# hzxie/Stereo-3D-Reconstruction

Hardware: NVIDIA B200
Metric: stereo pairs/sec Stereo2Voxel fwd (higher is better)
Workload: dtype bf16

## Files before the change

### include/s3d.h

```cpp
#ifndef S3D_H_
#define S3D_H_

#include <stdint.h>

#ifdef __cplusplus
extern "C" {
#endif

#define S3D_OK                0
#define S3D_ERR_INVALID      -1
#define S3D_ERR_CUDA         -2
#define S3D_ERR_UNSUPPORTED  -3

#define S3D_DTYPE_F32   0
#define S3D_DTYPE_BF16  1
#define S3D_DTYPE_BF16X2 2

#define S3D_ACT_NONE     0
#define S3D_ACT_RELU     1
#define S3D_ACT_LEAKY    2
#define S3D_ACT_SIGMOID  3
#define S3D_ACT_TANH     4

#define S3D_MAX_TAPS 64

typedef struct S3dConvParams {
  int32_t N, iD, iH, iW, Cin;
  int32_t oD, oH, oW, Cout;
  int32_t sz, sy, sx;
  int32_t ntaps, n_classes;
  int8_t  dz[S3D_MAX_TAPS], dy[S3D_MAX_TAPS], dx[S3D_MAX_TAPS];
  int64_t osN, osD, osH, osW;
  int64_t osC;
  int64_t os_lo;
  int32_t omz, omy, omx;
  int32_t cout_store;
  int32_t in_dtype, out_dtype;
  int32_t act;  float act_param;
  int32_t tw, th, td, tn;
  int32_t bn;
  const float* proj_w;
  int32_t proj_channel, proj_act;
  const void* w_nstack;
} S3dConvParams;

const char* s3d_version(void);
const char* s3d_last_error(void);
int s3d_device_check(int dev);
int s3d_set_knob(const char* name, int value);
int s3d_get_knob(const char* name);

int s3d_conv_igemm(const S3dConvParams* p, const void* in, const void* w, const float* bias,
                   const void* residual, void* out, void* stream);
int s3d_conv_direct(const S3dConvParams* p, const void* in, const void* w, const float* bias,
                    const void* residual, void* out, void* stream);

int s3d_conv2d_halo(const void* in, const void* w, const float* bias, const void* residual, void* out, int nimg, int h, int wd,
                    int cin, int cout, int64_t osN, int64_t osH, int64_t osW, int relu, void* stream);

int s3d_pack_image(const float* img, const float* disp, float disp_scale, void* out,
                   int B, int H, int W, int Cpad, int out_dtype, void* stream);

int s3d_pack_image_u8(const uint8_t* img, const float* disp, float disp_scale, float img_scale, void* out,
                      int B, int H, int W, int Cpad, int out_dtype, void* stream);

int s3d_conv_first(const void* img, int img_u8, const float* disp, float disp_scale, const void* w, const float* bias,
                   void* out, int B, int H, int W, int cin, int cin_pad, int cout_pad, int dtype, int act,
                   float act_param, void* stream);

int s3d_conv_concat_volume(const S3dConvParams* p, const void* feat, int feat_pitch, int feat_pad, const float* bias,
                           void* out, void* stream);
int s3d_conv_concat_volume_ro(const S3dConvParams* p, const void* feat, int feat_pitch, int feat_pad, const void* w_refonce,
                              const float* bias, void* out, void* stream);
int s3d_concat_gonce_assemble(const float* maps_l, const float* maps_r, const float* edge_l, const float* edge_r,
                              const float* bias, void* out, int B, int D, int h, int w, int map_w, int out_dtype, void* stream);
int s3d_map_conv(const void* in, const void* w, float* out, int nimg, int h, int in_w, int ow, int off, int ntx, int cout,
                 int dtype, void* stream);
int s3d_cost_volume_concat(const void* feat, void* vol, int B, int h, int w, int C, int D,
                           int dtype, void* stream);
int s3d_soft_argmin(const float* cost, float* disp, int N, int D, int h, int w, float sign,
                    void* stream);
int s3d_tap_gather_soft_argmin(const float* taps, float* disp, float* cost_out, int N, int D, int h, int w,
                               int tap_stride, float sign, void* stream);
int s3d_cls_soft_argmin(const void* x, const void* w_taps, float* disp, int N, int D, int h, int w, int C,
                        float sign, void* stream);
int64_t s3d_conv_cls_workspace_bytes(int N, int D, int h, int w);
int s3d_conv_cls_soft_argmin(const S3dConvParams* p, const void* in, const float* bias, const void* w_taps, void* workspace,
                             float* disp, float sign, void* stream);
int s3d_corr_soft_argmin(const void* feat, float* disp, float* cost_out, int B, int h, int w,
                         int C, int c_real, int D, int dtype, void* stream);
int s3d_upsample_disp(const float* disp_q, float* disp, int N, int h, int w, int H, int W,
                      float scale, void* stream);
int s3d_upsample_disp_eval(const float* disp_q, float* disp, const float* gt, const float* thresholds, int T,
                           float max_gt, long long* stats, int B, int h, int w, int H, int W, float scale, void* stream);
int s3d_upsample_disp_lr(const float* disp_q, float* disp, uint8_t* lr_mask, float lr_thresh, const float* gt,
                         const float* thresholds, int T, float max_gt, long long* disp_stats, long long* lr_stats,
                         int B, int h, int w, int H, int W, float scale, void* stream);

int s3d_latent_to_vox(const void* x, void* out, int N, int H, int W, int C, int L, int dtype,
                      void* stream);
int s3d_avg_pool(const void* x, void* out, int N, int H, int W, int C, int L, int dtype,
                 void* stream);
int s3d_depth_to_space(const void* in, void* out, const float* proj_w, int proj_act, int N, int d, int h, int w,
                       int Cpad, int dtype, void* stream);
int s3d_split_tf32(const float* x, float* hi, float* lo, int64_t n, void* stream);
int s3d_split_bf16(const float* x, void* out, int64_t npix, int C, void* stream);
int s3d_unsplit_bf16(const void* x, float* out, int64_t npix, int C, void* stream);
int s3d_fuse_views(const void* score, int64_t score_stride, const void* vol, int64_t vol_stride,
                   int dtype, float* fused, int B, int V, int nvox, const uint8_t* gt,
                   const float* thresholds, int T, long long* iou, int64_t score_lo, int64_t vol_lo, void* stream);

int s3d_chamfer_forward(const float* xyz1, const float* xyz2, float* dist1, int32_t* idx1,
                        float* dist2, int32_t* idx2, int B, int N, int M, void* stream);
int64_t s3d_chamfer_workspace_bytes(int B, int N, int M);
int s3d_chamfer_forward_ws(const float* xyz1, const float* xyz2, float* dist1, int32_t* idx1,
                           float* dist2, int32_t* idx2, int B, int N, int M, void* workspace,
                           int64_t workspace_bytes, void* stream);
int s3d_chamfer_eval(const float* xyz1, const float* xyz2, float* dist1, int32_t* idx1, float* dist2, int32_t* idx2,
                     int B, int N, int M, const float* tau, int T, long long* stats,
                     void* workspace, int64_t workspace_bytes, void* stream);

int s3d_fma_probe(float* sink, int iters, int64_t* fma_count, void* stream);

#ifdef __cplusplus
}
#endif
#endif
```

### stereo_3d_reconstruction_b200/csrc/common.cuh

```cuda
#pragma once
#include <cuda_runtime.h>
#include <cuda_bf16.h>
#include <stdint.h>
#include <stdio.h>
#include "../../include/s3d.h"

namespace s3d {

void set_error(const char* fmt, ...);

#define S3D_CHECK_ARG(cond, ...)                         \
  do {                                                   \
    if (!(cond)) {                                       \
      s3d::set_error(__VA_ARGS__);                       \
      return S3D_ERR_INVALID;                            \
    }                                                    \
  } while (0)

#define S3D_CUDA(expr)                                                              \
  do {                                                                              \
    cudaError_t _e = (expr);                                                        \
    if (_e != cudaSuccess) {                                                        \
      s3d::set_error("%s:%d %s -> %s", __FILE__, __LINE__, #expr, cudaGetErrorString(_e)); \
      return S3D_ERR_CUDA;                                                          \
    }                                                                               \
  } while (0)

#define S3D_LAUNCH_CHECK() S3D_CUDA(cudaGetLastError())

int num_sms();

struct Knobs {
  int no_scatter;
  int scatter_tps3;
  int scatter_no_pair;
  int scatter_ring;
  int scatter_res_transpose;
  int scatter_no_transpose;
  int scatter_generic;
  int no_corr_tc;
  int scatter_zsplit;
  int igemm_ts1;
  int igemm_one_cta;
  int scatter_one_cta;
  int no_conv_first_tc;
  int chamfer_sym;
  int chamfer_sym_r;
  int scatter_no_rm;
};
Knobs& knobs();

static inline int ceil_div(int a, int b) { return (a + b - 1) / b; }
static inline int64_t ceil_div64(int64_t a, int64_t b) { return (a + b - 1) / b; }

namespace {
constexpr int kMaxThresh = 8;
struct Thresh { float t[kMaxThresh]; };
}

template <typename T> __device__ __forceinline__ float to_f32(T v);
template <> __device__ __forceinline__ float to_f32<float>(float v) { return v; }
template <> __device__ __forceinline__ float to_f32<__nv_bfloat16>(__nv_bfloat16 v) { return __bfloat162float(v); }

template <typename T> __device__ __forceinline__ T from_f32(float v);
template <> __device__ __forceinline__ float from_f32<float>(float v) { return v; }
template <> __device__ __forceinline__ __nv_bfloat16 from_f32<__nv_bfloat16>(float v) { return __float2bfloat16_rn(v); }

__device__ __forceinline__ float fmax_nan(float a, float b) { float d; asm("max.NaN.f32 %0, %1, %2;" : "=f"(d) : "f"(a), "f"(b)); return d; }
__device__ __forceinline__ float fmin_nan(float a, float b) { float d; asm("min.NaN.f32 %0, %1, %2;" : "=f"(d) : "f"(a), "f"(b)); return d; }

__device__ __forceinline__ float apply_act(float v, int act, float a) {
  switch (act) {
    case S3D_ACT_RELU:    return fmax_nan(v, 0.f);
    case S3D_ACT_LEAKY:   return v > 0.f ? v : v * a;
    case S3D_ACT_SIGMOID: return 1.f / (1.f + expf(-v));
    case S3D_ACT_TANH:    return a * tanhf(v);
    default:              return v;
  }
}

static __device__ __noinline__ float apply_act_slow(float v, int act, float a) { return apply_act(v, act, a); }

}
```

### stereo_3d_reconstruction_b200/csrc/conv_scatter.cu

```cuda
#include "conv_scatter.cuh"

namespace s3d {
using namespace scatter;

bool conv_scatter_eligible(const S3dConvParams* p) {
  const int esz = p->in_dtype == S3D_DTYPE_F32 ? 4 : 2;
  const bool split = p->in_dtype == S3D_DTYPE_BF16X2;
  if (!p->w_nstack || knobs().no_scatter) return false;
  if (split && (p->out_dtype != S3D_DTYPE_BF16X2 || p->Cin > 64 || (p->Cout != 16 && p->Cout != 32 && p->Cout != 64) ||
                p->cout_store != p->Cout)) return false;
  if (!split && p->out_dtype == S3D_DTYPE_BF16X2) return false;
  if (p->n_classes != 1 || p->sx != 1 || p->sy != 1 || p->sz != 1 || p->ntaps != 27) return false;
  if (p->omx != 1 || p->omy != 1 || p->omz != 1 || p->osC != 1 || p->proj_w) return false;
  if (p->oD != p->iD || p->oH != p->iH || p->oW != p->iW) return false;
  for (int t = 0; t < 27; ++t)
    if (p->dz[t] != t / 9 - 1 || p->dy[t] != (t % 9) / 3 - 1 || p->dx[t] != t % 3 - 1) return false;
  const int cin_bytes = (split ? 2 : 1) * p->Cin * esz;
  if (split && cin_bytes == 32) return false;
  if (cin_bytes != 32 && cin_bytes != 64 && cin_bytes != 128 && cin_bytes != 256) return false;
  if (p->Cout > 64 || p->Cout % 16 != 0) return false;
  return true;
}

int conv_scatter_launch(const S3dConvParams* p_in, const void* in, const float* bias, const void* residual, void* out,
                        cudaStream_t stream) {
  const S3dConvParams& p = *p_in;
  const bool tf32 = p.in_dtype == S3D_DTYPE_F32;
  const bool split = p.in_dtype == S3D_DTYPE_BF16X2;
  const int esz = tf32 ? 4 : 2;
  const int cin_phys = split ? 2 * p.Cin : p.Cin;
  S3D_CHECK_ARG(p.cout_store >= 1 && p.cout_store <= p.Cout, "scatter: cout_store");
  ScArgs a;
  memset(&a, 0, sizeof(a));
  a.p = p;  a.bias = bias;  a.residual = residual;  a.out = out;
  a.split = split ? 1 : 0;
  a.os_lo = p.os_lo ? p.os_lo : (int64_t)p.Cout;
  a.nchunks = cin_phys * esz == 256 ? 2 : 1;
  a.row_bytes = cin_phys * esz / a.nchunks;
  a.kc = cin_phys / a.nchunks;
  a.chunk_stride = (kPlaneRows * a.row_bytes + 1023) / 1024 * 1024;
  a.slot_bytes = a.nchunks * a.chunk_stride;
  a.cp = p.Cout;
  a.tps = spec_tps(a.row_bytes, a.cp);
  if (knobs().scatter_tps3 && a.tps == 9) a.tps = 3;
  a.cols_x = ceil_div(p.oW, kTX);  a.cols_y = ceil_div(p.oH, kTY);
  int64_t total = (int64_t)p.N * a.cols_x * a.cols_y;
  S3D_CHECK_ARG(total > 0 && total < (1ll << 31), "scatter: column count out of range");
  a.nz = 1;  a.zc = p.oD;  a.dl = p.oD;
  {
    const int sms = num_sms();
    int nz = knobs().scatter_zsplit > 0 ? knobs().scatter_zsplit : (knobs().scatter_zsplit < 0 ? 1 : (int)(sms / total));
    if (nz > p.oD / 4) nz = p.oD / 4;
    if (nz > 1) {
      a.zc = ceil_div(p.oD, nz);
      a.nz = ceil_div(p.oD, a.zc);
      a.dl = a.zc + 2;
      if (a.nz > 1) total *= a.nz; else { a.nz = 1; a.zc = p.oD; a.dl = p.oD; }
    }
  }
  a.total_cols = (int)total;
  int grid = num_sms();
  a.pair = ((3 * a.cp / 2) % 8 == 0 && total >= 2 && grid >= 2 && !knobs().scatter_no_pair) ? 1 : 0;
  bool fast_ok;
  {
    const int oesz = p.out_dtype == S3D_DTYPE_F32 ? 4 : 2;
    const bool simple_act = p.act == S3D_ACT_NONE || p.act == S3D_ACT_RELU || p.act == S3D_ACT_LEAKY;
    auto aligned = [&](const void* q) { return (reinterpret_cast<uintptr_t>(q) & 15) == 0; };
    auto dense16 = [&](int64_t st) { return (st * oesz) % 16 == 0; };
    fast_ok = simple_act && bias != nullptr && p.cout_store == p.Cout && aligned(out) && aligned(residual) &&
              dense16(p.osW) && dense16(p.osH) && dense16(p.osD) && dense16(p.osN) && p.osW < (1ll << 24) &&
              (split || !knobs().scatter_no_transpose);
  }
  const bool two = fast_ok && a.pair && !tf32 && !split && a.nchunks == 1 && p.out_dtype == S3D_DTYPE_BF16 && residual == nullptr &&
                   spec_kernel(a.row_bytes, a.cp, false, p.act == S3D_ACT_RELU, true) != nullptr && total > grid &&
                   !knobs().scatter_generic && !knobs().scatter_one_cta && !knobs().scatter_tps3 && !knobs().scatter_ring;
  if (two) grid *= 2;
  if (a.pair) {
    if ((int64_t)grid > total) grid = (int)((total + 1) / 2 * 2);
    grid -= grid % 2;
    a.ncols_max = (int)((total + grid - 1) / grid);
  } else if ((int64_t)grid > total) grid = (int)total;
  const int w_rows = a.pair ? 3 * a.cp / 2 : 3 * a.cp;
  a.w_tx = a.tps * w_rows * a.row_bytes;
  a.w_bytes = (a.w_tx + 1023) / 1024 * 1024;
  const int budget = two ? 110 * 1024 : 227 * 1024 - 1024 - 512;
  int ring = (budget - 4 * a.w_bytes) / a.slot_bytes;
  if (ring > kMaxRing) ring = kMaxRing;
  if (ring < 2) ring = 2;
  if (a.row_bytes == 128 && ring > (a.pair && a.nchunks == 1 ? 3 : 2)) ring = a.pair && a.nchunks == 1 ? 3 : 2;
  if (const int r = knobs().scatter_ring) { if (r >= 2 && r <= kMaxRing) ring = r; }
  a.ring = ring;
  a.w_stages = (budget - a.ring * a.slot_bytes) / a.w_bytes;
  if (a.w_stages > kMaxW) a.w_stages = kMaxW;
  S3D_CHECK_ARG(a.w_stages >= 2, "scatter: not enough shared memory for the weight ring");
  a.idesc = ptx::make_instr_desc(tf32 ? 2 : 1, a.pair ? 256 : 128, 3 * a.cp);
  a.res_direct = !knobs().scatter_res_transpose;
  {
    auto dense16 = [&](int64_t st) { return (st * 2) % 16 == 0; };
    a.fast_store = fast_ok;
    if (split) {
      S3D_CHECK_ARG(a.fast_store && dense16(a.os_lo) && a.os_lo >= p.Cout,
                    "scatter (split operands): needs a bias, a none / ReLU / LeakyReLU activation and 16-byte aligned out / residual / strides");
      a.res_direct = 1;
    }
  }

  const CUtensorMapSwizzle sw = a.row_bytes == 128 ? CU_TENSOR_MAP_SWIZZLE_128B
                              : a.row_bytes == 64 ? CU_TENSOR_MAP_SWIZZLE_64B : CU_TENSOR_MAP_SWIZZLE_32B;
  CUtensorMap map_x, map_w;
  cuuint32_t box[5] = {(cuuint32_t)a.kc, kHX, kHY, 1, 1};
  cuuint32_t estr[5] = {1, 1, 1, 1, 1};
  int rc = encode_act_map(&map_x, in, esz, tf32, cin_phys, p.iW, p.iH, p.iD, p.N, box, estr, sw);
  if (rc != S3D_OK) return rc;
  rc = encode_weight_map(&map_w, p.w_nstack, esz, tf32, cin_phys, 3 * a.cp, 36, a.kc, w_rows, sw, a.tps);
  if (rc != S3D_OK) return rc;

  const bool rm = residual != nullptr && a.pair && !tf32 && !split && a.nchunks == 1 && a.row_bytes == 128 && a.cp == 64 &&
                  p.out_dtype == S3D_DTYPE_BF16 && a.fast_store && a.tps == 1 && (p.act == S3D_ACT_RELU || p.act == S3D_ACT_NONE) &&
                  p.osW == 64 && p.osH == (int64_t)p.oW * 64 && p.osD == (int64_t)p.oH * p.osH && p.osN == (int64_t)p.oD * p.osD &&
                  !knobs().scatter_no_rm && !knobs().scatter_generic;
  if (rm) {
    const int extra = kResBytes + 32 * 128;
    a.w_stages = (budget - a.ring * a.slot_bytes - extra) / a.w_bytes;
    if (a.w_stages > kMaxW) a.w_stages = kMaxW;
    S3D_CHECK_ARG(a.w_stages >= 3, "scatter: not enough shared memory for the residual stage");
    CUtensorMap map_r;
    cuuint32_t rbox[5] = {64, kTX, kTY, 1, 1};
    rc = encode_act_map(&map_r, residual, 2, false, 64, p.oW, p.oH, p.oD, p.N, rbox, estr, CU_TENSOR_MAP_SWIZZLE_128B);
    if (rc != S3D_OK) return rc;
    a.residual = nullptr;
    const int smem_rm = a.ring * a.slot_bytes + a.w_stages * a.w_bytes + extra + 1024;
    KernFnR kr = rm_kernel(p.act == S3D_ACT_RELU);
    S3D_CUDA(cudaFuncSetAttribute(kr, cudaFuncAttributeMaxDynamicSharedMemorySize, smem_rm));
    cudaLaunchConfig_t cfg;
    memset(&cfg, 0, sizeof(cfg));
    cfg.gridDim = dim3(grid);  cfg.blockDim = dim3(kThreads);  cfg.dynamicSmemBytes = smem_rm;  cfg.stream = stream;
    cudaLaunchAttribute attr;
    attr.id = cudaLaunchAttributeClusterDimension;
    attr.val.clusterDim.x = 2;  attr.val.clusterDim.y = 1;  attr.val.clusterDim.z = 1;
    cfg.attrs = &attr;  cfg.numAttrs = 1;
    S3D_CUDA(cudaLaunchKernelEx(&cfg, kr, map_x, map_w, map_r, a));
    S3D_LAUNCH_CHECK();
    return S3D_OK;
  }

  const int smem_bytes = a.ring * a.slot_bytes + a.w_stages * a.w_bytes + 1024;
  KernFn kern = a.pair ? (tf32 ? conv_scatter_kernel<true, true> : conv_scatter_kernel<false, true>)
                       : (tf32 ? conv_scatter_kernel<true, false> : conv_scatter_kernel<false, false>);
  if (split) {
    const bool lean = a.pair && a.tps == spec_tps(a.row_bytes, a.cp) && !knobs().scatter_generic;
    kern = split_kernel(lean, a.pair != 0, cin_phys * esz, a.cp, residual != nullptr, p.act == S3D_ACT_RELU);
  }
  else if (a.pair && !tf32 && a.nchunks == 1 && p.out_dtype == S3D_DTYPE_BF16 && a.fast_store && a.tps == spec_tps(a.row_bytes, a.cp) &&
      !knobs().scatter_generic) {
    const bool relu = p.act == S3D_ACT_RELU;
    if (KernFn k = spec_kernel(a.row_bytes, a.cp, residual != nullptr, relu, two && a.fast_store)) kern = k;
    else if (two) { set_error("scatter: the two-CTA kernel needs the coalesced store path"); return S3D_ERR_INVALID; }
  }
  S3D_CUDA(cudaFuncSetAttribute(kern, cudaFuncAttributeMaxDynamicSharedMemorySize, smem_bytes));
  if (a.pair) {
    cudaLaunchConfig_t cfg;
    memset(&cfg, 0, sizeof(cfg));
    cfg.gridDim = dim3(grid);  cfg.blockDim = dim3(kThreads);  cfg.dynamicSmemBytes = smem_bytes;  cfg.stream = stream;
    cudaLaunchAttribute attr;
    attr.id = cudaLaunchAttributeClusterDimension;
    attr.val.clusterDim.x = 2;  attr.val.clusterDim.y = 1;  attr.val.clusterDim.z = 1;
    cfg.attrs = &attr;  cfg.numAttrs = 1;
    S3D_CUDA(cudaLaunchKernelEx(&cfg, kern, map_x, map_w, a));
  } else {
    kern<<<grid, kThreads, smem_bytes, stream>>>(map_x, map_w, a);
  }
  S3D_LAUNCH_CHECK();
  return S3D_OK;
}

}
```

### stereo_3d_reconstruction_b200/csrc/conv_scatter.cuh

```cuda
#pragma once
#include <cuda.h>
#include <stdlib.h>
#include <string.h>
#include "common.cuh"
#include "ptx.cuh"
#include "epilogue.cuh"

namespace s3d {
namespace scatter {

constexpr int kThreads = 384;
constexpr int kTX = 8, kHX = kTX + 2;
constexpr int kTY = 32, kHY = kTY + 2;
constexpr int kTileY = 16;
constexpr int kPlaneRows = kHX * kHY;
constexpr int kMaxRing = 6;
constexpr int kMaxW = 12;
constexpr int kTmemCols = 512;
constexpr int kTileCols = 256;

struct ScArgs {
  S3dConvParams p;
  const float* bias;
  const void* residual;
  void* out;
  int row_bytes;
  int kc;
  int nchunks;
  int chunk_stride;
  int slot_bytes;
  int ring;
  int cp;
  int tps;
  int w_stages, w_bytes, w_tx;
  int cols_x, cols_y, total_cols;
  int pair;
  int ncols_max;
  uint32_t idesc;
  int fast_store;
  int res_direct;
  int split;
  int64_t os_lo;
  int nz, zc, dl;
};

struct ScCtrl {
  uint64_t plane_full[kMaxRing], plane_empty[kMaxRing];
  uint64_t w_full[kMaxW], w_empty[kMaxW];
  uint64_t acc_full[2], acc_empty[2];
  uint64_t res_full, res_empty;
  uint32_t tmem_base;
};

struct ScRes {
  const CUtensorMap* map_r;
  uint32_t res_u32;
  uint32_t ident_u32;
  uint32_t bar_rf, bar_re;
  uint32_t idesc_r;
  int cp;
};
constexpr int kResBytes = 256 * 128;

struct Col { int n, y0, x0, zb; };

__device__ __forceinline__ Col decode_col(const ScArgs& a, int c) {
  Col r;
  r.zb = 0;
  if (a.nz > 1) { r.zb = (c % a.nz) * a.zc - 1;  c /= a.nz; }
  r.x0 = (c % a.cols_x) * kTX;  c /= a.cols_x;
  r.y0 = (c % a.cols_y) * kTY;  c /= a.cols_y;
  r.n = c;
  return r;
}

__device__ __forceinline__ int cta_cols(const ScArgs& a) {
  return a.pair ? a.ncols_max : (a.total_cols - (int)blockIdx.x + (int)gridDim.x - 1) / (int)gridDim.x;
}

__device__ __forceinline__ uint64_t desc_hi(uint32_t sbo, int row_bytes) {
  const uint64_t layout = row_bytes == 128 ? 2ull : (row_bytes == 64 ? 4ull : 6ull);
  return (static_cast<uint64_t>(sbo >> 4) << 32) | (1ull << 46) | (layout << 61);
}
__device__ __forceinline__ uint32_t desc_lo(uint32_t addr) { return ((addr & 0x3FFFF) >> 4) | (1u << 16); }

template <int TPS, bool kPair, int NK = 1, bool kRM = false>
__device__ __forceinline__ void sc_produce(const ScArgs& a, ScCtrl& ctrl, uint32_t planes_u32, uint32_t w_u32,
                                           const CUtensorMap* map_x, const CUtensorMap* map_w, const ScRes* rs = nullptr) {
  constexpr int G = 9 * NK / TPS;
  const uint32_t bar_pf = ptx::smem_u32(&ctrl.plane_full[0]), bar_pe = ptx::smem_u32(&ctrl.plane_empty[0]);
  const uint32_t bar_wf = ptx::smem_u32(&ctrl.w_full[0]), bar_we = ptx::smem_u32(&ctrl.w_empty[0]);
  const int D = a.dl, ring = a.ring, w_stages = a.w_stages, ncols = cta_cols(a);
  const int slot_bytes = a.slot_bytes, w_bytes = a.w_bytes, w_tx = a.w_tx;
  const int crank = kPair ? (int)ptx::cluster_ctarank() : 0;
  const bool leader = crank == 0;
  const int w_row0 = kPair ? crank * (3 * a.cp / 2) : 0;
  const int plane_tx = NK * kPlaneRows * a.row_bytes;
  const int kc = a.kc, chunk_stride = a.chunk_stride;
  int ws = 0;  uint32_t wphase = 0;
  int pslot = 0;  uint32_t pphase = 0;
  int pci = 0, pj = 0, issued = 0;
  Col pc = decode_col(a, blockIdx.x);
  auto issue_plane = [&](bool blocking) -> bool {
    if (pci >= ncols) return false;
    const uint32_t be = bar_pe + 8 * pslot, bf = bar_pf + 8 * pslot;
    if (blocking) ptx::mbar_wait_u32(be, pphase ^ 1);
    else if (!ptx::mbar_test_wait_u32(be, pphase ^ 1)) return false;
    if (ptx::elect_one()) {
      if (kPair) {
        if (leader) ptx::mbar_arrive_expect_tx_u32(bf, 2 * plane_tx);
#pragma unroll
        for (int ch = 0; ch < NK; ++ch)
          ptx::tma_load_5d_2sm_u32(planes_u32 + pslot * slot_bytes + ch * chunk_stride, map_x, bf, ch * kc, pc.x0 - 1, pc.y0 - 1, pc.zb + pj, pc.n);
      } else {
        ptx::mbar_arrive_expect_tx_u32(bf, plane_tx);
#pragma unroll
        for (int ch = 0; ch < NK; ++ch)
          ptx::tma_load_5d_u32(planes_u32 + pslot * slot_bytes + ch * chunk_stride, map_x, bf, ch * kc, pc.x0 - 1, pc.y0 - 1, pc.zb + pj, pc.n);
      }
    }
    __syncwarp();
    ++issued;
    if (++pslot == ring) { pslot = 0; pphase ^= 1; }
    if (++pj == D) {
      pj = 0;  ++pci;
      if (pci < ncols) pc = decode_col(a, blockIdx.x + pci * gridDim.x);
    }
    return true;
  };
  int gp = 0;
  [[maybe_unused]] uint32_t rphase = 0;
  [[maybe_unused]] auto load_res = [&](const Col& rc, int p) {
    ptx::mbar_wait_u32(rs->bar_re, rphase ^ 1);
    if (ptx::elect_one()) {
      if (kPair) {
        if (leader) ptx::mbar_arrive_expect_tx_u32(rs->bar_rf, 2 * kResBytes);
        ptx::tma_load_5d_2sm_u32(rs->res_u32, rs->map_r, rs->bar_rf, 0, rc.x0, rc.y0, rc.zb + p, rc.n);
      } else {
        ptx::mbar_arrive_expect_tx_u32(rs->bar_rf, kResBytes);
        ptx::tma_load_5d_u32(rs->res_u32, rs->map_r, rs->bar_rf, 0, rc.x0, rc.y0, rc.zb + p, rc.n);
      }
    }
    __syncwarp();
    rphase ^= 1;
  };
  for (int ci = 0; ci < ncols; ++ci) {
    int rot = 3;
    [[maybe_unused]] const Col rc = decode_col(a, blockIdx.x + ci * gridDim.x);
    if constexpr (kRM) load_res(rc, 0);
    for (int p = 0; p < D; ++p, ++gp) {
      while (issued <= gp) issue_plane(true);
      const int ahead = gp + ring;
#pragma unroll
      for (int g = 0; g < G; ++g) {
        if (issued < ahead) issue_plane(false);
        const uint32_t be = bar_we + 8 * ws, bf = bar_wf + 8 * ws;
        ptx::mbar_wait_u32(be, wphase ^ 1);
        if (ptx::elect_one()) {
          const int tap = rot * 9 + (NK == 2 ? g / 2 : g * TPS), c0 = NK == 2 ? (g & 1) * kc : 0;
          if (kPair) {
            if (leader) ptx::mbar_arrive_expect_tx_u32(bf, 2 * w_tx);
            ptx::tma_load_3d_2sm_u32(w_u32 + ws * w_bytes, map_w, bf, c0, w_row0, tap);
          } else {
            ptx::mbar_arrive_expect_tx_u32(bf, w_tx);
            ptx::tma_load_3d_u32(w_u32 + ws * w_bytes, map_w, bf, c0, 0, tap);
          }
        }
        __syncwarp();
        if (++ws == w_stages) { ws = 0; wphase ^= 1; }
      }
      if constexpr (kRM) { if (p + 1 < D) load_res(rc, p + 1); }
      rot = (p == 0) ? 1 : (rot == 2 ? 0 : rot + 1);
    }
  }
}

struct ScIssue {
  uint32_t tmem_base, planes_u32, w_u32;
  uint32_t bar_pf, bar_pe, bar_wf, bar_we, bar_af, bar_ae;
  uint64_t x_hi, w_hi;
  int slot_bytes, w_bytes, w_stages, ring;
  uint32_t rb16, tap_step, tile_off, chunk_step;
  uint32_t idesc;
  int D, ncols;
};

template <bool kPair>
__device__ __forceinline__ void sc_commit(uint32_t bar) {
  if (kPair) ptx::tc_commit_2sm_u32(bar, 3);
  else       ptx::tc_commit_u32(bar);
}

template <bool kTF32, bool kPair>
__device__ __forceinline__ void sc_mma(uint32_t d_tmem, uint64_t ad, uint64_t bd, uint32_t idesc, uint32_t acc) {
  if (kPair) { if (kTF32) ptx::mma_tf32_2sm(d_tmem, ad, bd, idesc, acc); else ptx::mma_bf16_2sm(d_tmem, ad, bd, idesc, acc); }
  else       { if (kTF32) ptx::mma_tf32(d_tmem, ad, bd, idesc, acc);     else ptx::mma_bf16(d_tmem, ad, bd, idesc, acc); }
}

template <bool kTF32, int TPS, int kPer, bool kPair, int NK, bool kSplit>
__device__ __forceinline__ void sc_issue_group(const ScIssue& z, uint32_t d_tmem, uint64_t xdesc, uint64_t wdesc, int g,
                                               uint32_t first) {
#pragma unroll
  for (int tt = 0; tt < TPS; ++tt) {
    const int kyx = NK == 2 ? g / 2 : g * TPS + tt;
    const uint32_t xrow = ((kyx / 3) * kHX + (kyx % 3)) * z.rb16;
    if constexpr (!kSplit) {
      const uint32_t xoff = xrow + (NK == 2 ? (g & 1) * z.chunk_step : 0u);
#pragma unroll
      for (int k = 0; k < kPer; ++k) {
        const uint32_t acc = (g == 0 && tt == 0 && k == 0) ? first : 1u;
        sc_mma<kTF32, kPair>(d_tmem, xdesc + xoff + 2 * k, wdesc + tt * z.tap_step + 2 * k, z.idesc, acc);
      }
    } else if constexpr (NK == 2) {
      if ((g & 1) == 0) {
#pragma unroll
        for (int k = 0; k < kPer; ++k)
          sc_mma<kTF32, kPair>(d_tmem, xdesc + xrow + 2 * k, wdesc + 2 * k, z.idesc, (g == 0 && k == 0) ? first : 1u);
#pragma unroll
        for (int k = 0; k < kPer; ++k)
          sc_mma<kTF32, kPair>(d_tmem, xdesc + xrow + z.chunk_step + 2 * k, wdesc + 2 * k, z.idesc, 1u);
      } else {
#pragma unroll
        for (int k = 0; k < kPer; ++k)
          sc_mma<kTF32, kPair>(d_tmem, xdesc + xrow + 2 * k, wdesc + 2 * k, z.idesc, 1u);
      }
    } else {
      const uint64_t wd = wdesc + tt * z.tap_step;
#pragma unroll
      for (int k = 0; k < kPer; ++k)
        sc_mma<kTF32, kPair>(d_tmem, xdesc + xrow + 2 * k, wd + 2 * k, z.idesc, (g == 0 && tt == 0 && k == 0) ? first : 1u);
#pragma unroll
      for (int k = 0; k < kPer; ++k)
        sc_mma<kTF32, kPair>(d_tmem, xdesc + xrow + 2 * (kPer + k), wd + 2 * k, z.idesc, 1u);
#pragma unroll
      for (int k = 0; k < kPer; ++k)
        sc_mma<kTF32, kPair>(d_tmem, xdesc + xrow + 2 * k, wd + 2 * (kPer + k), z.idesc, 1u);
    }
  }
}

template <bool kPair, int CP>
__device__ __forceinline__ void sc_res_mma(const ScRes& rs, uint32_t d_tmem, uint64_t adesc, uint64_t idd) {
#pragma unroll
  for (int k = 0; k < CP / 16; ++k) sc_mma<false, kPair>(d_tmem, adesc + 2 * k, idd + 2 * k, rs.idesc_r, 1u);
}

template <bool kTF32, int TPS, int kPer, bool kPair, int NK = 1, bool kSplit = false, bool kRM = false, int kTP = kTileCols>
__device__ __forceinline__ void sc_issue(const ScIssue& z, const ScRes* rs = nullptr) {
  constexpr int G = 9 * NK / TPS;
  int ws = 0;  uint32_t wphase = 0;
  int pw = 0;  uint32_t pwphase = 0;
  uint32_t aphase = 0;
  [[maybe_unused]] uint32_t rphase = 0;
  [[maybe_unused]] uint64_t rdesc = 0, idd = 0;
  if constexpr (kRM) {
    const uint64_t hi = desc_hi(8 * 128, 128);
    rdesc = hi | desc_lo(rs->res_u32);
    idd = hi | desc_lo(rs->ident_u32);
  }
  const uint32_t w_lo0 = desc_lo(z.w_u32), w_lo_step = z.w_bytes >> 4;
  const uint32_t x_lo0 = desc_lo(z.planes_u32), x_lo_step = z.slot_bytes >> 4;
  const uint32_t d0 = z.tmem_base, d1 = z.tmem_base + kTP;
  for (int ci = 0; ci < z.ncols; ++ci) {
    for (int p = 0; p < z.D; ++p) {
      ptx::mbar_wait_u32(z.bar_pf + 8 * pw, pwphase);
      const uint64_t xd0 = z.x_hi | (x_lo0 + pw * x_lo_step);
      const uint64_t xd1 = xd0 + z.tile_off;
      const uint32_t first = p == 0 ? 0u : 1u;
      int ws_prev = 0;
#pragma unroll
      for (int g = 0; g <= G; ++g) {
        if (g < G) {
          ptx::mbar_wait_u32(z.bar_wf + 8 * ws, wphase);
          if (g == 0) ptx::mbar_wait_u32(z.bar_ae, aphase ^ 1);
          ptx::tc_fence_after();
          const uint64_t wd = z.w_hi | (w_lo0 + ws * w_lo_step);
          if constexpr (kRM) { if (g == G / 2) { ptx::mbar_wait_u32(rs->bar_rf, rphase); ptx::tc_fence_after(); } }
          if (ptx::elect_one()) {
            sc_issue_group<kTF32, TPS, kPer, kPair, NK, kSplit>(z, d0, xd0, wd, g, first);
            if constexpr (kRM) { if (g == G / 2) sc_res_mma<kPair, 64>(*rs, d0 + (uint32_t)(p % 3) * rs->cp, rdesc, idd); }
            if (g == G - 1) sc_commit<kPair>(z.bar_af);
          }
          __syncwarp();
        }
        if (g >= 1) {
          if (g == 1) { ptx::mbar_wait_u32(z.bar_ae + 8, aphase ^ 1); ptx::tc_fence_after(); }
          const uint64_t wd = z.w_hi | (w_lo0 + ws_prev * w_lo_step);
          if (ptx::elect_one()) {
            sc_issue_group<kTF32, TPS, kPer, kPair, NK, kSplit>(z, d1, xd1, wd, g - 1, first);
            sc_commit<kPair>(z.bar_we + 8 * ws_prev);
            if constexpr (kRM) {
              if (g == G / 2 + 1) {
                sc_res_mma<kPair, 64>(*rs, d1 + (uint32_t)(p % 3) * rs->cp, rdesc + (128 * 128 >> 4), idd);
                sc_commit<kPair>(rs->bar_re);
              }
            }
            if (g == G) { sc_commit<kPair>(z.bar_af + 8); sc_commit<kPair>(z.bar_pe + 8 * pw); }
          }
          __syncwarp();
        }
        if (g < G) {
          ws_prev = ws;
          if (++ws == z.w_stages) { ws = 0; wphase ^= 1; }
        }
      }
      aphase ^= 1;
      if constexpr (kRM) rphase ^= 1;
      if (++pw == z.ring) { pw = 0; pwphase ^= 1; }
    }
  }
}

template <int NCH>
__device__ __forceinline__ void chunk_transpose(uint4 (&c)[NCH], int lane) {
#pragma unroll
  for (int s = NCH / 2; s >= 1; s >>= 1) {
    const bool up = (lane & s) != 0;
#pragma unroll
    for (int a = 0; a < NCH; ++a) {
      if (a & s) continue;
      const uint4 send = up ? c[a] : c[a | s];
      uint4 recv;
      recv.x = __shfl_xor_sync(0xffffffffu, send.x, s);
      recv.y = __shfl_xor_sync(0xffffffffu, send.y, s);
      recv.z = __shfl_xor_sync(0xffffffffu, send.z, s);
      recv.w = __shfl_xor_sync(0xffffffffu, send.w, s);
      if (up) c[a] = recv; else c[a | s] = recv;
    }
  }
}

struct ScEpi {
  const float* bias;  const void* residual;  void* out;
  float slope;
  int osW;
  int res_direct;
};

template <int NCH, typename TOut>
__device__ __forceinline__ void sc_res_load(const ScEpi& e, int64_t grp_off, int osW, int lane, uint32_t okmask, uint4 (&r)[NCH]) {
  const int j = lane & (NCH - 1);
  if (e.res_direct) {
    const int own = (lane & 7) & (NCH - 1);
    const TOut* rs = reinterpret_cast<const TOut*>(e.residual) + grp_off + own * osW;
    const bool ok = (okmask >> own) & 1u;
#pragma unroll
    for (int k = 0; k < NCH; ++k)
      r[k] = ok ? __ldg(reinterpret_cast<const uint4*>(rs) + k) : make_uint4(0, 0, 0, 0);
    return;
  }
  const TOut* rs = reinterpret_cast<const TOut*>(e.residual) + grp_off + j * (16 / (int)sizeof(TOut));
#pragma unroll
  for (int k = 0; k < NCH; ++k)
    r[k] = ((okmask >> k) & 1u) ? __ldg(reinterpret_cast<const uint4*>(rs + k * osW)) : make_uint4(0, 0, 0, 0);
}

template <int CP, typename TOut, bool kRes, int kAct>
__device__ __forceinline__ void sc_fast_store(const ScEpi& e, int64_t grp_off, int lane, uint32_t okmask,
                                              const uint32_t (&v)[CP / 16][16], uint4 (&r)[CP * sizeof(TOut) / 16]) {
  constexpr int NCH = CP * sizeof(TOut) / 16;
  constexpr int CPC = 16 / sizeof(TOut);
  uint4 c[NCH];
  if (kRes && !e.res_direct) chunk_transpose<NCH>(r, lane);
#pragma unroll
  for (int jg = 0; jg < CP / 16; ++jg) {
    float f[16];
    const float4* b4 = reinterpret_cast<const float4*>(e.bias + 16 * jg);
#pragma unroll
    for (int i = 0; i < 4; ++i) {
      const float4 b = __ldg(b4 + i);
      f[4 * i] = __uint_as_float(v[jg][4 * i]) + b.x;          f[4 * i + 1] = __uint_as_float(v[jg][4 * i + 1]) + b.y;
      f[4 * i + 2] = __uint_as_float(v[jg][4 * i + 2]) + b.z;  f[4 * i + 3] = __uint_as_float(v[jg][4 * i + 3]) + b.w;
    }
    if (kRes) {
      if (sizeof(TOut) == 2) {
#pragma unroll
        for (int h = 0; h < 2; ++h) {
          const __nv_bfloat162* hp = reinterpret_cast<const __nv_bfloat162*>(&r[2 * jg + h]);
#pragma unroll
          for (int i = 0; i < 4; ++i) {
            const float2 g = __bfloat1622float2(hp[i]);
            f[8 * h + 2 * i] += g.x;  f[8 * h + 2 * i + 1] += g.y;
          }
        }
      } else {
#pragma unroll
        for (int h = 0; h < 4; ++h) {
          const float4 g = *reinterpret_cast<const float4*>(&r[4 * jg + h]);
          f[4 * h] += g.x;  f[4 * h + 1] += g.y;  f[4 * h + 2] += g.z;  f[4 * h + 3] += g.w;
        }
      }
    }
#pragma unroll
    for (int i = 0; i < 16; ++i) f[i] = kAct == 0 ? fmax_nan(f[i], 0.f) : (kAct == 1 ? f[i] : fmax_nan(f[i], 0.f) + e.slope * fmin_nan(f[i], 0.f));
    if (sizeof(TOut) == 2) {
#pragma unroll
      for (int h = 0; h < 2; ++h) {
        __nv_bfloat162* hp = reinterpret_cast<__nv_bfloat162*>(&c[2 * jg + h]);
#pragma unroll
        for (int i = 0; i < 4; ++i) hp[i] = __floats2bfloat162_rn(f[8 * h + 2 * i], f[8 * h + 2 * i + 1]);
      }
    } else {
#pragma unroll
      for (int h = 0; h < 4; ++h) c[4 * jg + h] = *reinterpret_cast<const uint4*>(&f[4 * h]);
    }
  }
  chunk_transpose<NCH>(c, lane);
  const int j = lane & (NCH - 1);
  TOut* o = reinterpret_cast<TOut*>(e.out) + grp_off + j * CPC;
#pragma unroll
  for (int k = 0; k < NCH; ++k)
    if ((okmask >> k) & 1u) *reinterpret_cast<uint4*>(o + k * e.osW) = c[k];
}

template <int CP, typename TOut>
__device__ __forceinline__ void sc_fast_plane(const ScEpi& e, int64_t grp_off, int lane, uint32_t okmask,
                                              const uint32_t (&v)[CP / 16][16], uint4 (&r)[CP * sizeof(TOut) / 16]) {
  if (e.slope == 0.f) {
    if (e.residual) sc_fast_store<CP, TOut, true, 0>(e, grp_off, lane, okmask, v, r);
    else            sc_fast_store<CP, TOut, false, 0>(e, grp_off, lane, okmask, v, r);
  } else {
    if (e.residual) sc_fast_store<CP, TOut, true, 2>(e, grp_off, lane, okmask, v, r);
    else            sc_fast_store<CP, TOut, false, 2>(e, grp_off, lane, okmask, v, r);
  }
}

template <int CP, typename TOut, bool kFast, int kSRes = -1, int kSAct = -1, int kTP = kTileCols>
__device__ __forceinline__ void sc_epilogue(const ScArgs& a, ScCtrl& ctrl, uint32_t tmem_base, int warp, int lane) {
  constexpr int NCH = kFast ? CP * (int)sizeof(TOut) / 16 : 1;
  const int t = (warp - 4) >> 2, q = warp & 3;
  const EpiParams ep = {a.bias, a.residual, a.out, a.p.cout_store, sizeof(TOut) == 2, a.p.act, a.p.act_param, 1, nullptr, 0, 0};
  const ScEpi fe = {a.bias, a.residual, a.out,
                    a.p.act == S3D_ACT_NONE ? 1.f : (a.p.act == S3D_ACT_LEAKY ? a.p.act_param : 0.f), (int)a.p.osW, a.res_direct};
  const uint32_t bar_af = ptx::smem_u32(&ctrl.acc_full[t]), bar_ae = ptx::smem_u32(&ctrl.acc_empty[t]);
  const uint32_t tbase = tmem_base + t * kTP + (static_cast<uint32_t>(q * 32) << 16);
  const int yl = t * kTileY + q * 4 + (lane >> 3), xl = lane & 7;
  const int D = a.dl;
  const int zs0 = a.nz > 1 ? 1 : 0, zs1 = a.nz > 1 ? a.zc + 1 : D;
  const int xb = xl & ~(NCH - 1);
  uint32_t aphase = 0;
  const int ncols = cta_cols(a);
  for (int ci = 0; ci < ncols; ++ci) {
    const Col c = decode_col(a, blockIdx.x + ci * gridDim.x);
    const bool rowok = c.y0 + yl < a.p.oH && c.n < a.p.N;
    const bool ok = rowok && c.x0 + xl < a.p.oW;
    const int64_t row_off = (int64_t)c.n * a.p.osN + (int64_t)(c.y0 + yl) * a.p.osH + (int64_t)c.x0 * a.p.osW;
    const int64_t pix_off = row_off + (int64_t)xl * a.p.osW;
    const int64_t grp_off = row_off + (int64_t)xb * a.p.osW;
    uint32_t okmask = 0;
#pragma unroll
    for (int k = 0; k < NCH; ++k) okmask |= (rowok && c.x0 + xb + k < a.p.oW) ? (1u << k) : 0u;
    int slot = 0, z = 0;
    for (int p = 0; p < D; ++p) {
      const int ndrain = (p >= 1 ? 1 : 0) + (p == D - 1 ? 1 : 0);
      uint4 r[NCH];
      if constexpr (kFast) {
        if (a.residual && ndrain)
          sc_res_load<NCH, TOut>(fe, grp_off + (int64_t)(c.zb + z) * a.p.osD, fe.osW, lane,
                                 (z >= zs0 && z < zs1 && c.zb + z < a.p.oD) ? okmask : 0u, r);
      }
      ptx::mbar_wait_u32(bar_af, aphase);
      ptx::tc_fence_after();
      if (ndrain == 0) {
        ptx::tc_fence_before();
        __syncwarp();
        if (lane == 0) { if (a.pair) ptx::mbar_arrive_cluster_u32(bar_ae, 0); else ptx::mbar_arrive_u32(bar_ae); }
      }
      for (int i = 0; i < ndrain; ++i) {
        uint32_t v[CP / 16][16];
        const uint32_t taddr = tbase + slot * CP;
#pragma unroll
        for (int j = 0; j < CP / 16; ++j) ptx::tmem_ld16(taddr + 16 * j, v[j]);
        ptx::tmem_ld_wait();
#pragma unroll
        for (int j = 0; j < CP / 16; ++j) ptx::tmem_st16_zero(taddr + 16 * j);
        ptx::tmem_st_wait();
        if (i == ndrain - 1) {
          ptx::tc_fence_before();
          __syncwarp();
          if (lane == 0) { if (a.pair) ptx::mbar_arrive_cluster_u32(bar_ae, 0); else ptx::mbar_arrive_u32(bar_ae); }
        }
        const int64_t zo = (int64_t)(c.zb + z) * a.p.osD;
        const bool stz = z >= zs0 && z < zs1 && c.zb + z < a.p.oD;
        const uint32_t om = stz ? okmask : 0u;
        if constexpr (kFast) {
          if (i == 1 && a.residual) sc_res_load<NCH, TOut>(fe, grp_off + zo, fe.osW, lane, om, r);
          if constexpr (kSRes >= 0) sc_fast_store<CP, TOut, kSRes != 0, kSAct>(fe, grp_off + zo, lane, om, v, r);
          else sc_fast_plane<CP, TOut>(fe, grp_off + zo, lane, om, v, r);
        } else {
          if (ok && stz) {
#pragma unroll
            for (int j = 0; j < CP / 16; ++j) epilogue_store16(ep, pix_off + zo, 16 * j, v[j]);
          }
        }
        ++z;
        if (++slot == 3) slot = 0;
      }
      aphase ^= 1;
    }
  }
}

template <int CP>
__device__ __forceinline__ void sc_epilogue_dispatch(const ScArgs& a, ScCtrl& ctrl, uint32_t tmem_base, int warp, int lane) {
  constexpr bool kPow2_16 = CP == 16 || CP == 32 || CP == 64;
  constexpr bool kPow2_32 = CP == 16 || CP == 32;
  if (a.p.out_dtype == S3D_DTYPE_BF16) {
    if (kPow2_16 && a.fast_store) sc_epilogue<CP, __nv_bfloat16, kPow2_16>(a, ctrl, tmem_base, warp, lane);
    else sc_epilogue<CP, __nv_bfloat16, false>(a, ctrl, tmem_base, warp, lane);
  } else {
    if (kPow2_32 && a.fast_store) sc_epilogue<CP, float, kPow2_32>(a, ctrl, tmem_base, warp, lane);
    else sc_epilogue<CP, float, false>(a, ctrl, tmem_base, warp, lane);
  }
}

template <int NCH>
__device__ __forceinline__ void sc_res_load_split(const ScEpi& e, int64_t os_lo, int64_t grp_off, int lane, uint32_t okmask,
                                                  uint4 (&rh)[NCH], uint4 (&rl)[NCH]) {
  const int own = (lane & 7) & (NCH - 1);
  const __nv_bfloat16* rs = reinterpret_cast<const __nv_bfloat16*>(e.residual) + grp_off + (int64_t)own * e.osW;
  const bool ok = (okmask >> own) & 1u;
#pragma unroll
  for (int k = 0; k < NCH; ++k) {
    rh[k] = ok ? __ldg(reinterpret_cast<const uint4*>(rs) + k) : make_uint4(0, 0, 0, 0);
    rl[k] = ok ? __ldg(reinterpret_cast<const uint4*>(rs + os_lo) + k) : make_uint4(0, 0, 0, 0);
  }
}

template <int CP, bool kRes, int kAct>
__device__ __forceinline__ void sc_split_store(const ScEpi& e, int64_t os_lo, int64_t grp_off, int lane, uint32_t okmask,
                                               uint32_t (&v)[CP / 16][16], const uint4 (&rh)[CP / 8], const uint4 (&rl)[CP / 8]) {
  constexpr int NCH = CP / 8;
#pragma unroll
  for (int jg = 0; jg < CP / 16; ++jg) {
    const float4* b4 = reinterpret_cast<const float4*>(e.bias + 16 * jg);
#pragma unroll
    for (int i = 0; i < 4; ++i) {
      const float4 b = __ldg(b4 + i);
      float f0 = __uint_as_float(v[jg][4 * i]) + b.x, f1 = __uint_as_float(v[jg][4 * i + 1]) + b.y;
      float f2 = __uint_as_float(v[jg][4 * i + 2]) + b.z, f3 = __uint_as_float(v[jg][4 * i + 3]) + b.w;
      if (kRes) {
        const __nv_bfloat162* ph = reinterpret_cast<const __nv_bfloat162*>(&rh[2 * jg + (i >> 1)]) + 2 * (i & 1);
        const __nv_bfloat162* pl = reinterpret_cast<const __nv_bfloat162*>(&rl[2 * jg + (i >> 1)]) + 2 * (i & 1);
        const float2 h0 = __bfloat1622float2(ph[0]), h1 = __bfloat1622float2(ph[1]);
        const float2 l0 = __bfloat1622float2(pl[0]), l1 = __bfloat1622float2(pl[1]);
        f0 += h0.x + l0.x;  f1 += h0.y + l0.y;  f2 += h1.x + l1.x;  f3 += h1.y + l1.y;
      }
      if (kAct == 0) { f0 = fmax_nan(f0, 0.f); f1 = fmax_nan(f1, 0.f); f2 = fmax_nan(f2, 0.f); f3 = fmax_nan(f3, 0.f); }
      else if (kAct == 2) {
        f0 = fmax_nan(f0, 0.f) + e.slope * fmin_nan(f0, 0.f);  f1 = fmax_nan(f1, 0.f) + e.slope * fmin_nan(f1, 0.f);
        f2 = fmax_nan(f2, 0.f) + e.slope * fmin_nan(f2, 0.f);  f3 = fmax_nan(f3, 0.f) + e.slope * fmin_nan(f3, 0.f);
      }
      v[jg][4 * i] = __float_as_uint(f0);      v[jg][4 * i + 1] = __float_as_uint(f1);
      v[jg][4 * i + 2] = __float_as_uint(f2);  v[jg][4 * i + 3] = __float_as_uint(f3);
    }
  }
  const int j = lane & (NCH - 1);
  __nv_bfloat16* o = reinterpret_cast<__nv_bfloat16*>(e.out) + grp_off + j * 8;
#pragma unroll
  for (int half = 0; half < 2; ++half) {
    uint4 c[NCH];
#pragma unroll
    for (int jg = 0; jg < CP / 16; ++jg) {
#pragma unroll
      for (int h = 0; h < 2; ++h) {
        uint32_t w[4];
#pragma unroll
        for (int i = 0; i < 4; ++i) {
          uint32_t hi, lo;
          split_bf16x2(__uint_as_float(v[jg][8 * h + 2 * i]), __uint_as_float(v[jg][8 * h + 2 * i + 1]), hi, lo);
          w[i] = half == 0 ? hi : lo;
        }
        c[2 * jg + h] = make_uint4(w[0], w[1], w[2], w[3]);
      }
    }
    chunk_transpose<NCH>(c, lane);
    __nv_bfloat16* oh = o + (half == 0 ? (int64_t)0 : os_lo);
#pragma unroll
    for (int k = 0; k < NCH; ++k)
      if ((okmask >> k) & 1u) *reinterpret_cast<uint4*>(oh + k * e.osW) = c[k];
  }
}

template <int CP, int kSRes = -1, int kSAct = -1>
__device__ __forceinline__ void sc_epilogue_split(const ScArgs& a, ScCtrl& ctrl, uint32_t tmem_base, int warp, int lane) {
  constexpr int NCH = CP / 8;
  const int t = (warp - 4) >> 2, q = warp & 3;
  const ScEpi fe = {a.bias, a.residual, a.out,
                    a.p.act == S3D_ACT_NONE ? 1.f : (a.p.act == S3D_ACT_LEAKY ? a.p.act_param : 0.f), (int)a.p.osW, 1};
  const int64_t os_lo = a.os_lo;
  const uint32_t bar_af = ptx::smem_u32(&ctrl.acc_full[t]), bar_ae = ptx::smem_u32(&ctrl.acc_empty[t]);
  const uint32_t tbase = tmem_base + t * kTileCols + (static_cast<uint32_t>(q * 32) << 16);
  const int yl = t * kTileY + q * 4 + (lane >> 3), xl = lane & 7;
  const int D = a.dl;
  const int zs0 = a.nz > 1 ? 1 : 0, zs1 = a.nz > 1 ? a.zc + 1 : D;
  const int xb = xl & ~(NCH - 1);
  uint32_t aphase = 0;
  const int ncols = cta_cols(a);
  for (int ci = 0; ci < ncols; ++ci) {
    const Col c = decode_col(a, blockIdx.x + ci * gridDim.x);
    const bool rowok = c.y0 + yl < a.p.oH && c.n < a.p.N;
    const int64_t row_off = (int64_t)c.n * a.p.osN + (int64_t)(c.y0 + yl) * a.p.osH + (int64_t)c.x0 * a.p.osW;
    const int64_t grp_off = row_off + (int64_t)xb * a.p.osW;
    uint32_t okmask = 0;
#pragma unroll
    for (int k = 0; k < NCH; ++k) okmask |= (rowok && c.x0 + xb + k < a.p.oW) ? (1u << k) : 0u;
    int slot = 0, z = 0;
    for (int p = 0; p < D; ++p) {
      const int ndrain = (p >= 1 ? 1 : 0) + (p == D - 1 ? 1 : 0);
      uint4 rh[NCH], rl[NCH];
      if (a.residual && ndrain)
        sc_res_load_split<NCH>(fe, os_lo, grp_off + (int64_t)(c.zb + z) * a.p.osD, lane,
                               (z >= zs0 && z < zs1 && c.zb + z < a.p.oD) ? okmask : 0u, rh, rl);
      ptx::mbar_wait_u32(bar_af, aphase);
      ptx::tc_fence_after();
      if (ndrain == 0) {
        ptx::tc_fence_before();
        __syncwarp();
        if (lane == 0) { if (a.pair) ptx::mbar_arrive_cluster_u32(bar_ae, 0); else ptx::mbar_arrive_u32(bar_ae); }
      }
      for (int i = 0; i < ndrain; ++i) {
        uint32_t v[CP / 16][16];
        const uint32_t taddr = tbase + slot * CP;
#pragma unroll
        for (int j = 0; j < CP / 16; ++j) ptx::tmem_ld16(taddr + 16 * j, v[j]);
        ptx::tmem_ld_wait();
#pragma unroll
        for (int j = 0; j < CP / 16; ++j) ptx::tmem_st16_zero(taddr + 16 * j);
        ptx::tmem_st_wait();
        if (i == ndrain - 1) {
          ptx::tc_fence_before();
          __syncwarp();
          if (lane == 0) { if (a.pair) ptx::mbar_arrive_cluster_u32(bar_ae, 0); else ptx::mbar_arrive_u32(bar_ae); }
        }
        const int64_t zo = (int64_t)(c.zb + z) * a.p.osD;
        const uint32_t om = (z >= zs0 && z < zs1 && c.zb + z < a.p.oD) ? okmask : 0u;
        if (i == 1 && a.residual) sc_res_load_split<NCH>(fe, os_lo, grp_off + zo, lane, om, rh, rl);
        if constexpr (kSRes >= 0) {
          sc_split_store<CP, kSRes != 0, kSAct>(fe, os_lo, grp_off + zo, lane, om, v, rh, rl);
        } else if (fe.slope == 0.f) {
          if (a.residual) sc_split_store<CP, true, 0>(fe, os_lo, grp_off + zo, lane, om, v, rh, rl);
          else            sc_split_store<CP, false, 0>(fe, os_lo, grp_off + zo, lane, om, v, rh, rl);
        } else {
          if (a.residual) sc_split_store<CP, true, 2>(fe, os_lo, grp_off + zo, lane, om, v, rh, rl);
          else            sc_split_store<CP, false, 2>(fe, os_lo, grp_off + zo, lane, om, v, rh, rl);
        }
        ++z;
        if (++slot == 3) slot = 0;
      }
      aphase ^= 1;
    }
  }
}

__host__ __device__ constexpr int spec_tps(int rb, int cp) {
  return rb == 128 ? 1 : (9 * (3 * cp / 2) * rb <= 28 * 1024 ? 9 : 3);
}

template <bool kTF32, bool kPair, int RB = 0, int CP = 0, int kSRes = -1, int kSAct = -1, bool kSplit = false, bool kTwo = false>
__global__ void __launch_bounds__(kThreads, kTwo ? 2 : 1)
conv_scatter_kernel(const __grid_constant__ CUtensorMap map_x, const __grid_constant__ CUtensorMap map_w,
                    const __grid_constant__ ScArgs a) {
  extern __shared__ uint8_t smem_raw[];
  uint8_t* smem = reinterpret_cast<uint8_t*>((reinterpret_cast<uintptr_t>(smem_raw) + 1023) & ~uintptr_t(1023));
  uint8_t* smem_w = smem + a.ring * a.slot_bytes;
  __shared__ ScCtrl ctrl;
  const int warp = threadIdx.x >> 5;
  const int lane = threadIdx.x & 31;

  if (warp == 0 && lane == 0) {
    ptx::prefetch_tensormap(&map_x);
    ptx::prefetch_tensormap(&map_w);
  }
  if (warp == 1 && lane == 0) {
    for (int s = 0; s < kMaxRing; ++s) { ptx::mbar_init(&ctrl.plane_full[s], 1); ptx::mbar_init(&ctrl.plane_empty[s], 1); }
    for (int s = 0; s < kMaxW; ++s) { ptx::mbar_init(&ctrl.w_full[s], 1); ptx::mbar_init(&ctrl.w_empty[s], 1); }
    for (int b = 0; b < 2; ++b) { ptx::mbar_init(&ctrl.acc_full[b], 1); ptx::mbar_init(&ctrl.acc_empty[b], kPair ? 8 : 4); }
    ptx::fence_barrier_init();
  }
  constexpr int kTP = kTwo ? 128 : kTileCols;
  if (warp == 2) { if (kPair) ptx::tmem_alloc_2sm(&ctrl.tmem_base, 2 * kTP); else ptx::tmem_alloc(&ctrl.tmem_base, 2 * kTP); }
  ptx::tc_fence_before();
  __syncthreads();
  if (kPair) ptx::cluster_sync_all();
  ptx::tc_fence_after();
  const uint32_t tmem_base = ctrl.tmem_base;

  if (warp == 0) {
    const uint32_t planes_u32 = ptx::smem_u32(smem), w_u32 = ptx::smem_u32(smem_w);
    if constexpr (RB == 256) sc_produce<1, kPair, 2>(a, ctrl, planes_u32, w_u32, &map_x, &map_w);
    else if constexpr (RB == 128) sc_produce<1, kPair>(a, ctrl, planes_u32, w_u32, &map_x, &map_w);
    else if constexpr (RB != 0) sc_produce<spec_tps(RB, CP), kPair>(a, ctrl, planes_u32, w_u32, &map_x, &map_w);
    else if (a.nchunks == 2) sc_produce<1, kPair, 2>(a, ctrl, planes_u32, w_u32, &map_x, &map_w);
    else if (a.tps == 1) sc_produce<1, kPair>(a, ctrl, planes_u32, w_u32, &map_x, &map_w);
    else if (a.tps == 3) sc_produce<3, kPair>(a, ctrl, planes_u32, w_u32, &map_x, &map_w);
    else sc_produce<9, kPair>(a, ctrl, planes_u32, w_u32, &map_x, &map_w);
  } else if (warp == 1 && (!kPair || ptx::cluster_ctarank() == 0)) {
    const int rb = a.row_bytes;
    const ScIssue zi = {tmem_base, ptx::smem_u32(smem), ptx::smem_u32(smem_w),
                        ptx::smem_u32(&ctrl.plane_full[0]), ptx::smem_u32(&ctrl.plane_empty[0]), ptx::smem_u32(&ctrl.w_full[0]),
                        ptx::smem_u32(&ctrl.w_empty[0]), ptx::smem_u32(&ctrl.acc_full[0]), ptx::smem_u32(&ctrl.acc_empty[0]),
                        desc_hi(kHX * rb, rb), desc_hi(8 * rb, rb), a.slot_bytes, a.w_bytes, a.w_stages, a.ring,
                        (uint32_t)(rb >> 4), (uint32_t)(((kPair ? 3 * a.cp / 2 : 3 * a.cp) * rb) >> 4), (uint32_t)((kTileY * kHX * rb) >> 4), (uint32_t)(a.chunk_stride >> 4), a.idesc,
                        a.dl, cta_cols(a)};
    if constexpr (kSplit) {
      if constexpr (RB == 256) sc_issue<false, 1, 4, kPair, 2, true>(zi);
      else if constexpr (RB == 128) sc_issue<false, 1, 2, kPair, 1, true>(zi);
      else if constexpr (RB == 64) sc_issue<false, spec_tps(RB, CP), 1, kPair, 1, true>(zi);
      else if (a.nchunks == 2) sc_issue<false, 1, 4, kPair, 2, true>(zi);
      else if (rb == 128) sc_issue<false, 1, 2, kPair, 1, true>(zi);
      else if (a.tps == 9) sc_issue<false, 9, 1, kPair, 1, true>(zi);
      else sc_issue<false, 3, 1, kPair, 1, true>(zi);
    }
    else if constexpr (RB == 128) sc_issue<kTF32, 1, 4, kPair>(zi);
    else if constexpr (RB == 64) sc_issue<kTF32, spec_tps(RB, CP), 2, kPair>(zi);
    else if constexpr (RB == 32) sc_issue<kTF32, spec_tps(RB, CP), 1, kPair, 1, false, false, kTP>(zi);
    else if (a.nchunks == 2) sc_issue<kTF32, 1, 4, kPair, 2>(zi);
    else if (rb == 128) sc_issue<kTF32, 1, 4, kPair>(zi);
    else if (rb == 64 && a.tps == 9) sc_issue<kTF32, 9, 2, kPair>(zi);
    else if (rb == 64) sc_issue<kTF32, 3, 2, kPair>(zi);
    else if (a.tps == 3) sc_issue<kTF32, 3, 1, kPair>(zi);
    else sc_issue<kTF32, 9, 1, kPair>(zi);
  } else if (warp >= 4) {
    if constexpr (kSplit) {
      if constexpr (RB != 0) sc_epilogue_split<CP, kSRes, kSAct>(a, ctrl, tmem_base, warp, lane);
      else if (a.cp == 64) sc_epilogue_split<64>(a, ctrl, tmem_base, warp, lane);
      else if (a.cp == 32) sc_epilogue_split<32>(a, ctrl, tmem_base, warp, lane);
      else sc_epilogue_split<16>(a, ctrl, tmem_base, warp, lane);
    }
    else if constexpr (RB != 0) sc_epilogue<CP, __nv_bfloat16, true, kSRes, kSAct, kTP>(a, ctrl, tmem_base, warp, lane);
    else if (a.cp == 64) sc_epilogue_dispatch<64>(a, ctrl, tmem_base, warp, lane);
    else if (a.cp == 48) sc_epilogue_dispatch<48>(a, ctrl, tmem_base, warp, lane);
    else if (a.cp == 32) sc_epilogue_dispatch<32>(a, ctrl, tmem_base, warp, lane);
    else sc_epilogue_dispatch<16>(a, ctrl, tmem_base, warp, lane);
  }

  ptx::tc_fence_before();
  __syncthreads();
  if (kPair) ptx::cluster_sync_all();
  if (warp == 2) {
    ptx::tc_fence_after();
    if (kPair) ptx::tmem_dealloc_2sm(tmem_base, 2 * kTP); else ptx::tmem_dealloc(tmem_base, 2 * kTP);
  }
}


typedef void (*KernFn)(CUtensorMap, CUtensorMap, ScArgs);
KernFn spec_kernel(int row_bytes, int cp, bool residual, bool relu, bool two_ctas = false);
KernFn split_kernel(bool lean, bool pair, int phys_row_bytes, int cp, bool residual, bool relu);
typedef void (*KernFnR)(CUtensorMap, CUtensorMap, CUtensorMap, ScArgs);
KernFnR rm_kernel(bool relu);

}
}
```

### stereo_3d_reconstruction_b200/csrc/conv_scatter_rm.cu

```cuda
#include "conv_scatter.cuh"

namespace s3d {
namespace scatter {

template <int kSAct>
__global__ void __launch_bounds__(kThreads, 1)
conv_scatter_rm_kernel(const __grid_constant__ CUtensorMap map_x, const __grid_constant__ CUtensorMap map_w,
                       const __grid_constant__ CUtensorMap map_r, const __grid_constant__ ScArgs a) {
  constexpr bool kPair = true;
  constexpr int CP = 64;
  extern __shared__ uint8_t smem_raw[];
  uint8_t* smem = reinterpret_cast<uint8_t*>((reinterpret_cast<uintptr_t>(smem_raw) + 1023) & ~uintptr_t(1023));
  uint8_t* smem_w = smem + a.ring * a.slot_bytes;
  uint8_t* smem_res = smem_w + a.w_stages * a.w_bytes;
  uint8_t* smem_id = smem_res + kResBytes;
  __shared__ ScCtrl ctrl;
  const int warp = threadIdx.x >> 5;
  const int lane = threadIdx.x & 31;

  if (warp == 0 && lane == 0) {
    ptx::prefetch_tensormap(&map_x);
    ptx::prefetch_tensormap(&map_w);
    ptx::prefetch_tensormap(&map_r);
  }
  if (warp == 1 && lane == 0) {
    for (int s = 0; s < kMaxRing; ++s) { ptx::mbar_init(&ctrl.plane_full[s], 1); ptx::mbar_init(&ctrl.plane_empty[s], 1); }
    for (int s = 0; s < kMaxW; ++s) { ptx::mbar_init(&ctrl.w_full[s], 1); ptx::mbar_init(&ctrl.w_empty[s], 1); }
    for (int b = 0; b < 2; ++b) { ptx::mbar_init(&ctrl.acc_full[b], 1); ptx::mbar_init(&ctrl.acc_empty[b], 8); }
    ptx::mbar_init(&ctrl.res_full, 1);  ptx::mbar_init(&ctrl.res_empty, 1);
    ptx::fence_barrier_init();
  }
  if (warp == 2) ptx::tmem_alloc_2sm(&ctrl.tmem_base, kTmemCols);
  if (warp == 3) {
    uint4* z4 = reinterpret_cast<uint4*>(smem_id);
    for (int i = lane; i < (CP / 2) * 128 / 16; i += 32) z4[i] = make_uint4(0, 0, 0, 0);
    __syncwarp();
    const int r = lane, ci = (int)ptx::cluster_ctarank() * (CP / 2) + lane;
    *reinterpret_cast<__nv_bfloat16*>(smem_id + (r >> 3) * 1024 + (r & 7) * 128 + (((ci >> 3) ^ (r & 7)) << 4) + (ci & 7) * 2) =
        __float2bfloat16_rn(1.f);
    ptx::fence_proxy_async();
  }
  ptx::tc_fence_before();
  __syncthreads();
  ptx::cluster_sync_all();
  ptx::tc_fence_after();
  const uint32_t tmem_base = ctrl.tmem_base;
  const ScRes rs = {&map_r, ptx::smem_u32(smem_res), ptx::smem_u32(smem_id), ptx::smem_u32(&ctrl.res_full),
                    ptx::smem_u32(&ctrl.res_empty), ptx::make_instr_desc(1, 256, CP), CP};

  if (warp == 0) {
    sc_produce<1, kPair, 1, true>(a, ctrl, ptx::smem_u32(smem), ptx::smem_u32(smem_w), &map_x, &map_w, &rs);
  } else if (warp == 1 && ptx::cluster_ctarank() == 0) {
    const int rb = a.row_bytes;
    const ScIssue zi = {tmem_base, ptx::smem_u32(smem), ptx::smem_u32(smem_w),
                        ptx::smem_u32(&ctrl.plane_full[0]), ptx::smem_u32(&ctrl.plane_empty[0]), ptx::smem_u32(&ctrl.w_full[0]),
                        ptx::smem_u32(&ctrl.w_empty[0]), ptx::smem_u32(&ctrl.acc_full[0]), ptx::smem_u32(&ctrl.acc_empty[0]),
                        desc_hi(kHX * rb, rb), desc_hi(8 * rb, rb), a.slot_bytes, a.w_bytes, a.w_stages, a.ring,
                        (uint32_t)(rb >> 4), (uint32_t)(((3 * a.cp / 2) * rb) >> 4), (uint32_t)((kTileY * kHX * rb) >> 4),
                        (uint32_t)(a.chunk_stride >> 4), a.idesc, a.dl, cta_cols(a)};
    sc_issue<false, 1, 4, kPair, 1, false, true>(zi, &rs);
  } else if (warp >= 4) {
    sc_epilogue<CP, __nv_bfloat16, true, 0, kSAct>(a, ctrl, tmem_base, warp, lane);
  }

  ptx::tc_fence_before();
  __syncthreads();
  ptx::cluster_sync_all();
  if (warp == 2) {
    ptx::tc_fence_after();
    ptx::tmem_dealloc_2sm(tmem_base, kTmemCols);
  }
}

KernFnR rm_kernel(bool relu) { return relu ? conv_scatter_rm_kernel<0> : conv_scatter_rm_kernel<2>; }

}
}
```

### stereo_3d_reconstruction_b200/csrc/voxel.cu

```cuda
#include <stdarg.h>
#include <stdlib.h>
#include <string.h>
#include "common.cuh"

namespace s3d {

static thread_local char g_err[512] = "";
void set_error(const char* fmt, ...) {
  va_list ap;
  va_start(ap, fmt);
  vsnprintf(g_err, sizeof(g_err), fmt, ap);
  va_end(ap);
}
int num_sms() {
  int dev = 0, n = 0;
  if (cudaGetDevice(&dev) != cudaSuccess || cudaDeviceGetAttribute(&n, cudaDevAttrMultiProcessorCount, dev) != cudaSuccess || n <= 0)
    n = 148;
  return n;
}

namespace {
struct KnobName { const char* name; const char* env; int Knobs::*field; };
const KnobName kKnobNames[] = {
    {"no_scatter", "S3D_NO_SCATTER", &Knobs::no_scatter},
    {"scatter_tps3", "S3D_SCATTER_TPS3", &Knobs::scatter_tps3},
    {"scatter_no_pair", "S3D_SCATTER_NO_PAIR", &Knobs::scatter_no_pair},
    {"scatter_ring", "S3D_SCATTER_RING", &Knobs::scatter_ring},
    {"scatter_res_transpose", "S3D_SCATTER_RES_TRANSPOSE", &Knobs::scatter_res_transpose},
    {"scatter_no_transpose", "S3D_SCATTER_NO_TRANSPOSE", &Knobs::scatter_no_transpose},
    {"scatter_generic", "S3D_SCATTER_GENERIC", &Knobs::scatter_generic},
    {"no_corr_tc", "S3D_NO_CORR_TC", &Knobs::no_corr_tc},
    {"scatter_zsplit", "S3D_SCATTER_ZSPLIT", &Knobs::scatter_zsplit},
    {"scatter_no_rm", "S3D_SCATTER_NO_RM", &Knobs::scatter_no_rm},
    {"igemm_ts1", "S3D_IGEMM_TS1", &Knobs::igemm_ts1},
    {"no_conv_first_tc", "S3D_NO_CONV_FIRST_TC", &Knobs::no_conv_first_tc},
    {"scatter_one_cta", "S3D_SCATTER_ONE_CTA", &Knobs::scatter_one_cta},
    {"igemm_one_cta", "S3D_IGEMM_ONE_CTA", &Knobs::igemm_one_cta},
    {"chamfer_sym", "S3D_CHAMFER_SYM", &Knobs::chamfer_sym},
    {"chamfer_sym_r", "S3D_CHAMFER_SYM_R", &Knobs::chamfer_sym_r},
};
}

Knobs& knobs() {
  static Knobs k = [] {
    Knobs v;
    memset(&v, 0, sizeof(v));
    for (const KnobName& n : kKnobNames)
      if (const char* e = getenv(n.env)) { const int x = atoi(e); v.*(n.field) = x != 0 ? x : 1; }
    return v;
  }();
  return k;
}

namespace {

template <typename T>
__global__ void pack_image_kernel(const float* __restrict__ img, const float* __restrict__ disp, float disp_scale,
                                  T* __restrict__ out, int B, int H, int W, int Cpad) {
  const int64_t plane = (int64_t)H * W, total = plane * B;
  for (int64_t i = blockIdx.x * (int64_t)blockDim.x + threadIdx.x; i < total; i += (int64_t)gridDim.x * blockDim.x) {
    const int64_t b = i / plane, pix = i % plane;
    const float* ip = img + b * 3 * plane + pix;
    const float c0 = ip[0], c1 = ip[plane], c2 = ip[2 * plane], c3 = disp ? disp[i] * disp_scale : 0.f;
    T* o = out + i * Cpad;
    if (sizeof(T) == 2 && (Cpad & 7) == 0) {
      uint4 v0 = make_uint4(0, 0, 0, 0);
      __nv_bfloat162 p01 = __floats2bfloat162_rn(c0, c1), p23 = __floats2bfloat162_rn(c2, c3);
      v0.x = *reinterpret_cast<uint32_t*>(&p01);
      v0.y = *reinterpret_cast<uint32_t*>(&p23);
      uint4* o4 = reinterpret_cast<uint4*>(o);
      o4[0] = v0;
      for (int c = 1; c < Cpad / 8; ++c) o4[c] = make_uint4(0, 0, 0, 0);
    } else if (sizeof(T) == 4 && (Cpad & 3) == 0) {
      float4* o4 = reinterpret_cast<float4*>(o);
      o4[0] = make_float4(c0, c1, c2, c3);
      for (int c = 1; c < Cpad / 4; ++c) o4[c] = make_float4(0.f, 0.f, 0.f, 0.f);
    } else {
      o[0] = from_f32<T>(c0);  o[1] = from_f32<T>(c1);  o[2] = from_f32<T>(c2);  o[3] = from_f32<T>(c3);
      for (int c = 4; c < Cpad; ++c) o[c] = from_f32<T>(0.f);
    }
  }
}

template <typename T>
__global__ void pack_image_u8_kernel(const uint8_t* __restrict__ img, const float* __restrict__ disp, float disp_scale,
                                     float img_scale, T* __restrict__ out, int64_t total, int Cpad) {
  for (int64_t i = blockIdx.x * (int64_t)blockDim.x + threadIdx.x; i < total; i += (int64_t)gridDim.x * blockDim.x) {
    const uint8_t* ip = img + i * 3;
    const float c0 = (float)ip[0] * img_scale, c1 = (float)ip[1] * img_scale, c2 = (float)ip[2] * img_scale;
    const float c3 = disp ? disp[i] * disp_scale : 0.f;
    T* o = out + i * Cpad;
    if (sizeof(T) == 2 && (Cpad & 7) == 0) {
      uint4 v0 = make_uint4(0, 0, 0, 0);
      __nv_bfloat162 p01 = __floats2bfloat162_rn(c0, c1), p23 = __floats2bfloat162_rn(c2, c3);
      v0.x = *reinterpret_cast<uint32_t*>(&p01);
      v0.y = *reinterpret_cast<uint32_t*>(&p23);
      uint4* o4 = reinterpret_cast<uint4*>(o);
      o4[0] = v0;
      for (int c = 1; c < Cpad / 8; ++c) o4[c] = make_uint4(0, 0, 0, 0);
    } else {
      o[0] = from_f32<T>(c0);  o[1] = from_f32<T>(c1);  o[2] = from_f32<T>(c2);  o[3] = from_f32<T>(c3);
      for (int c = 4; c < Cpad; ++c) o[c] = from_f32<T>(0.f);
    }
  }
}

__device__ __forceinline__ void pool_bin(int i, int in, int out, int& s, int& e) {
  s = (i * in) / out;
  e = ((i + 1) * in + out - 1) / out;
}

template <typename T>
__global__ void pool_kernel(const T* __restrict__ x, T* __restrict__ out, int N, int H, int W, int C, int L, int to_vox) {
  const int64_t total = (int64_t)N * L * L * C;
  const int K = C * L * L / 8;
  for (int64_t i = blockIdx.x * (int64_t)blockDim.x + threadIdx.x; i < total; i += (int64_t)gridDim.x * blockDim.x) {
    int64_t r = i;
    const int c = (int)(r % C);  r /= C;
    const int px = (int)(r % L);  r /= L;
    const int py = (int)(r % L);  r /= L;
    const int n = (int)r;
    int ys, ye, xs, xe;
    pool_bin(py, H, L, ys, ye);
    pool_bin(px, W, L, xs, xe);
    float acc = 0.f;
    for (int yy = ys; yy < ye; ++yy)
      for (int xx = xs; xx < xe; ++xx) acc += to_f32(x[(((int64_t)n * H + yy) * W + xx) * C + c]);
    acc /= (float)((ye - ys) * (xe - xs));
    if (to_vox) {
      const int f = (c * L + py) * L + px;
      const int k = f >> 3, cell = f & 7;
      out[((int64_t)n * 8 + cell) * K + k] = from_f32<T>(acc);
    } else {
      out[i] = from_f32<T>(acc);
    }
  }
}

__global__ void pool_split_kernel(const __nv_bfloat16* __restrict__ x, __nv_bfloat16* __restrict__ out, int N, int H, int W, int C,
                                  int L, int to_vox) {
  const int64_t total = (int64_t)N * L * L * C;
  const int K = C * L * L / 8;
  for (int64_t i = blockIdx.x * (int64_t)blockDim.x + threadIdx.x; i < total; i += (int64_t)gridDim.x * blockDim.x) {
    int64_t r = i;
    const int c = (int)(r % C);  r /= C;
    const int px = (int)(r % L);  r /= L;
    const int py = (int)(r % L);  r /= L;
    const int n = (int)r;
    int ys, ye, xs, xe;
    pool_bin(py, H, L, ys, ye);
    pool_bin(px, W, L, xs, xe);
    float acc = 0.f;
    for (int yy = ys; yy < ye; ++yy)
      for (int xx = xs; xx < xe; ++xx) {
        const __nv_bfloat16* q = x + (((int64_t)n * H + yy) * W + xx) * 2 * C + c;
        acc += __bfloat162float(q[0]) + __bfloat162float(q[C]);
      }
    acc /= (float)((ye - ys) * (xe - xs));
    const __nv_bfloat16 hi = __float2bfloat16_rn(acc), lo = __float2bfloat16_rn(acc - __bfloat162float(hi));
    if (to_vox) {
      const int f = (c * L + py) * L + px;
      const int k = f >> 3, cell = f & 7;
      __nv_bfloat16* o = out + ((int64_t)n * 8 + cell) * 2 * K + k;
      o[0] = hi;  o[K] = lo;
    } else {
      __nv_bfloat16* o = out + (i / C) * 2 * C + c;
      o[0] = hi;  o[C] = lo;
    }
  }
}

template <typename T>
__global__ void __launch_bounds__(256)
fuse_views_kernel(const T* __restrict__ score, int64_t sstride, const T* __restrict__ vol, int64_t vstride,
                  float* __restrict__ fused, int B, int V, int nvox, const uint8_t* __restrict__ gt, Thresh th, int nT,
                  unsigned long long* __restrict__ iou, int64_t score_lo, int64_t vol_lo) {
  auto ld = [](const T* p, int64_t lo) { return lo ? to_f32(p[0]) + to_f32(p[lo]) : to_f32(p[0]); };
  const int b = blockIdx.y;
  unsigned inter[kMaxThresh], uni[kMaxThresh];
#pragma unroll
  for (int t = 0; t < kMaxThresh; ++t) { inter[t] = 0; uni[t] = 0; }
  for (int i = blockIdx.x * blockDim.x + threadIdx.x; i < nvox; i += gridDim.x * blockDim.x) {
    float m = -INFINITY;
    for (int v = 0; v < V; ++v) m = fmaxf(m, ld(score + (((int64_t)v * B + b) * nvox + i) * sstride, score_lo));
    float s = 0.f, acc = 0.f;
    for (int v = 0; v < V; ++v) {
      const int64_t e = ((int64_t)v * B + b) * nvox + i;
      const float w = expf(ld(score + e * sstride, score_lo) - m);
      s += w;
      acc += w * ld(vol + e * vstride, vol_lo);
    }
    float f = acc / s;
    f = fminf(fmaxf(f, 0.f), 1.f);
    fused[(int64_t)b * nvox + i] = f;
    if (gt) {
      const bool g = gt[(int64_t)b * nvox + i] != 0;
#pragma unroll
      for (int t = 0; t < kMaxThresh; ++t)
        if (t < nT) { const bool p = f >= th.t[t]; inter[t] += (p && g); uni[t] += (p || g); }
    }
  }
  if (gt && iou) {
    __shared__ unsigned blk[2 * kMaxThresh];
    if (threadIdx.x < 2 * kMaxThresh) blk[threadIdx.x] = 0;
    __syncthreads();
#pragma unroll
    for (int t = 0; t < kMaxThresh; ++t) {
      if (t >= nT) break;
      unsigned a = inter[t], u = uni[t];
      for (int o = 16; o > 0; o >>= 1) { a += __shfl_xor_sync(0xffffffffu, a, o); u += __shfl_xor_sync(0xffffffffu, u, o); }
      if ((threadIdx.x & 31) == 0) {
        if (a) atomicAdd(&blk[2 * t], a);
        if (u) atomicAdd(&blk[2 * t + 1], u);
      }
    }
    __syncthreads();
    if ((int)threadIdx.x < 2 * nT && blk[threadIdx.x])
      atomicAdd(iou + (int64_t)b * nT * 2 + threadIdx.x, (unsigned long long)blk[threadIdx.x]);
  }
}

int grid_for(int64_t total, int threads) {
  int64_t blocks = ceil_div64(total, threads);
  const int64_t cap = (int64_t)num_sms() * 16;
  return (int)(blocks > cap ? cap : (blocks < 1 ? 1 : blocks));
}

}
}

using namespace s3d;

extern "C" const char* s3d_version(void) { return "s3d_b200 0.1 (sm_100a)"; }
extern "C" const char* s3d_last_error(void) { return g_err; }

extern "C" int s3d_set_knob(const char* name, int value) {
  if (!name) { set_error("s3d_set_knob: null name"); return S3D_ERR_INVALID; }
  for (const KnobName& n : kKnobNames)
    if (strcmp(name, n.name) == 0) { knobs().*(n.field) = value; return S3D_OK; }
  set_error("s3d_set_knob: unknown knob '%s'", name);
  return S3D_ERR_INVALID;
}
extern "C" int s3d_get_knob(const char* name) {
  if (name)
    for (const KnobName& n : kKnobNames)
      if (strcmp(name, n.name) == 0) return knobs().*(n.field);
  set_error("s3d_get_knob: unknown knob");
  return S3D_ERR_INVALID;
}

extern "C" int s3d_device_check(int dev) {
  cudaDeviceProp prop;
  cudaError_t e = cudaGetDeviceProperties(&prop, dev);
  if (e != cudaSuccess) { set_error("s3d_device_check: %s", cudaGetErrorString(e)); cudaGetLastError(); return S3D_ERR_CUDA; }
  if (prop.major != 10) { set_error("s3d_device_check: device %d is sm_%d%d, need sm_100", dev, prop.major, prop.minor); return S3D_ERR_UNSUPPORTED; }
  return S3D_OK;
}

extern "C" int s3d_pack_image(const float* img, const float* disp, float disp_scale, void* out, int B, int H, int W,
                              int Cpad, int out_dtype, void* stream) {
  if (!img || !out) { set_error("pack_image: null argument"); return S3D_ERR_INVALID; }
  S3D_CHECK_ARG(B > 0 && H > 0 && W > 0 && Cpad >= 4, "pack_image: bad shape");
  cudaStream_t st = static_cast<cudaStream_t>(stream);
  const int64_t total = (int64_t)B * H * W;
  if (out_dtype == S3D_DTYPE_BF16)
    pack_image_kernel<__nv_bfloat16><<<grid_for(total, 256), 256, 0, st>>>(img, disp, disp_scale, static_cast<__nv_bfloat16*>(out), B, H, W, Cpad);
  else if (out_dtype == S3D_DTYPE_F32)
    pack_image_kernel<float><<<grid_for(total, 256), 256, 0, st>>>(img, disp, disp_scale, static_cast<float*>(out), B, H, W, Cpad);
  else { set_error("pack_image: bad dtype"); return S3D_ERR_INVALID; }
  S3D_LAUNCH_CHECK();
  return S3D_OK;
}

extern "C" int s3d_pack_image_u8(const uint8_t* img, const float* disp, float disp_scale, float img_scale, void* out,
                                 int B, int H, int W, int Cpad, int out_dtype, void* stream) {
  if (!img || !out) { set_error("pack_image_u8: null argument"); return S3D_ERR_INVALID; }
  S3D_CHECK_ARG(B > 0 && H > 0 && W > 0 && Cpad >= 4, "pack_image_u8: bad shape");
  cudaStream_t st = static_cast<cudaStream_t>(stream);
  const int64_t total = (int64_t)B * H * W;
  if (out_dtype == S3D_DTYPE_BF16)
    pack_image_u8_kernel<__nv_bfloat16><<<grid_for(total, 256), 256, 0, st>>>(img, disp, disp_scale, img_scale, static_cast<__nv_bfloat16*>(out), total, Cpad);
  else if (out_dtype == S3D_DTYPE_F32)
    pack_image_u8_kernel<float><<<grid_for(total, 256), 256, 0, st>>>(img, disp, disp_scale, img_scale, static_cast<float*>(out), total, Cpad);
  else { set_error("pack_image_u8: bad dtype"); return S3D_ERR_INVALID; }
  S3D_LAUNCH_CHECK();
  return S3D_OK;
}

template <typename T>
__global__ void depth_to_space_kernel(const T* __restrict__ in, T* __restrict__ out, const float* __restrict__ proj_w,
                                      int proj_act, int N, int d, int h, int w, int Cpad) {
  const int64_t total = (int64_t)N * d * h * w * 8;
  float pw[8];
#pragma unroll
  for (int c = 0; c < 8; ++c) pw[c] = proj_w ? __ldg(proj_w + c) : 0.f;
  for (int64_t i = blockIdx.x * (int64_t)blockDim.x + threadIdx.x; i < total; i += (int64_t)gridDim.x * blockDim.x) {
    const int cls = (int)(i & 7);
    int64_t r = i >> 3;
    const int x = (int)(r % w);  r /= w;
    const int y = (int)(r % h);  r /= h;
    const int z = (int)(r % d);  r /= d;
    const int n = (int)r;
    float f[8];
    const T* ip = in + i * 8;
    const int oz = 2 * z + (cls >> 2), oy = 2 * y + ((cls >> 1) & 1), ox = 2 * x + (cls & 1);
    T* op = out + ((((int64_t)n * 2 * d + oz) * 2 * h + oy) * 2 * w + ox) * Cpad;
    if (sizeof(T) == 2 && Cpad == 16) {
      const uint4 raw = __ldg(reinterpret_cast<const uint4*>(ip));
      const __nv_bfloat162* hp = reinterpret_cast<const __nv_bfloat162*>(&raw);
      float pr = 0.f;
#pragma unroll
      for (int c = 0; c < 4; ++c) {
        const float2 g = __bfloat1622float2(hp[c]);
        pr = fmaf(g.x, pw[2 * c], pr);  pr = fmaf(g.y, pw[2 * c + 1], pr);
      }
      uint4 hi = make_uint4(0, 0, 0, 0);
      const __nv_bfloat16 pb = __float2bfloat16_rn(proj_w ? apply_act(pr, proj_act, 1.f) : 0.f);
      hi.x = (uint32_t)(*reinterpret_cast<const unsigned short*>(&pb));
      reinterpret_cast<uint4*>(op)[0] = raw;
      reinterpret_cast<uint4*>(op)[1] = hi;
      continue;
    }
    if (sizeof(T) == 4 && Cpad == 16) {
      const float4 a = __ldg(reinterpret_cast<const float4*>(ip)), b = __ldg(reinterpret_cast<const float4*>(ip) + 1);
      float pr = a.x * pw[0];
      pr = fmaf(a.y, pw[1], pr);  pr = fmaf(a.z, pw[2], pr);  pr = fmaf(a.w, pw[3], pr);
      pr = fmaf(b.x, pw[4], pr);  pr = fmaf(b.y, pw[5], pr);  pr = fmaf(b.z, pw[6], pr);  pr = fmaf(b.w, pw[7], pr);
      float4* o4 = reinterpret_cast<float4*>(op);
      o4[0] = a;  o4[1] = b;
      o4[2] = make_float4(proj_w ? apply_act(pr, proj_act, 1.f) : 0.f, 0.f, 0.f, 0.f);
      o4[3] = make_float4(0.f, 0.f, 0.f, 0.f);
      continue;
    }
#pragma unroll
    for (int c = 0; c < 8; ++c) f[c] = to_f32(ip[c]);
#pragma unroll
    for (int c = 0; c < 8; ++c) op[c] = from_f32<T>(f[c]);
    if (Cpad > 8) {
      float pr = 0.f;
#pragma unroll
      for (int c = 0; c < 8; ++c) pr = fmaf(f[c], pw[c], pr);
      op[8] = from_f32<T>(proj_w ? apply_act(pr, proj_act, 1.f) : 0.f);
      for (int c = 9; c < Cpad; ++c) op[c] = from_f32<T>(0.f);
    }
  }
}

__global__ void depth_to_space_split_kernel(const __nv_bfloat16* __restrict__ in, __nv_bfloat16* __restrict__ out,
                                            const float* __restrict__ proj_w, int proj_act, int N, int d, int h, int w) {
  const int64_t total = (int64_t)N * d * h * w * 8;
  float pw[8];
#pragma unroll
  for (int c = 0; c < 8; ++c) pw[c] = proj_w ? __ldg(proj_w + c) : 0.f;
  for (int64_t i = blockIdx.x * (int64_t)blockDim.x + threadIdx.x; i < total; i += (int64_t)gridDim.x * blockDim.x) {
    const int cls = (int)(i & 7);
    int64_t r = i >> 3;
    const int64_t pix = r;
    const int x = (int)(r % w);  r /= w;
    const int y = (int)(r % h);  r /= h;
    const int z = (int)(r % d);  r /= d;
    const int n = (int)r;
    const __nv_bfloat16* ip = in + pix * 128 + cls * 8;
    const uint4 rh = __ldg(reinterpret_cast<const uint4*>(ip)), rl = __ldg(reinterpret_cast<const uint4*>(ip + 64));
    const __nv_bfloat162* ph = reinterpret_cast<const __nv_bfloat162*>(&rh);
    const __nv_bfloat162* pl = reinterpret_cast<const __nv_bfloat162*>(&rl);
    float pr = 0.f;
#pragma unroll
    for (int c = 0; c < 4; ++c) {
      const float2 gh = __bfloat1622float2(ph[c]), gl = __bfloat1622float2(pl[c]);
      pr = fmaf(gh.x + gl.x, pw[2 * c], pr);  pr = fmaf(gh.y + gl.y, pw[2 * c + 1], pr);
    }
    pr = proj_w ? apply_act(pr, proj_act, 1.f) : 0.f;
    const __nv_bfloat16 prh = __float2bfloat16_rn(pr), prl = __float2bfloat16_rn(pr - __bfloat162float(prh));
    const int oz = 2 * z + (cls >> 2), oy = 2 * y + ((cls >> 1) & 1), ox = 2 * x + (cls & 1);
    __nv_bfloat16* op = out + ((((int64_t)n * 2 * d + oz) * 2 * h + oy) * 2 * w + ox) * 32;
    uint4 zh = make_uint4(0, 0, 0, 0), zl = make_uint4(0, 0, 0, 0);
    zh.x = (uint32_t)(*reinterpret_cast<const unsigned short*>(&prh));
    zl.x = (uint32_t)(*reinterpret_cast<const unsigned short*>(&prl));
    reinterpret_cast<uint4*>(op)[0] = rh;  reinterpret_cast<uint4*>(op)[1] = zh;
    reinterpret_cast<uint4*>(op)[2] = rl;  reinterpret_cast<uint4*>(op)[3] = zl;
  }
}

extern "C" int s3d_depth_to_space(const void* in, void* out, const float* proj_w, int proj_act, int N, int d, int h, int w,
                                  int Cpad, int dtype, void* stream) {
  if (!in || !out) { set_error("depth_to_space: null argument"); return S3D_ERR_INVALID; }
  S3D_CHECK_ARG(N > 0 && d > 0 && h > 0 && w > 0 && Cpad >= 8 && (Cpad == 8 || Cpad >= 9), "depth_to_space: bad shape");
  cudaStream_t st = static_cast<cudaStream_t>(stream);
  const int64_t total = (int64_t)N * d * h * w * 8;
  if (dtype == S3D_DTYPE_BF16X2) {
    S3D_CHECK_ARG(Cpad == 16, "depth_to_space (split): Cpad must be 16");
    depth_to_space_split_kernel<<<grid_for(total, 256), 256, 0, st>>>(static_cast<const __nv_bfloat16*>(in),
        static_cast<__nv_bfloat16*>(out), proj_w, proj_act, N, d, h, w);
  } else if (dtype == S3D_DTYPE_BF16)
    depth_to_space_kernel<__nv_bfloat16><<<grid_for(total, 256), 256, 0, st>>>(static_cast<const __nv_bfloat16*>(in),
        static_cast<__nv_bfloat16*>(out), proj_w, proj_act, N, d, h, w, Cpad);
  else if (dtype == S3D_DTYPE_F32)
    depth_to_space_kernel<float><<<grid_for(total, 256), 256, 0, st>>>(static_cast<const float*>(in), static_cast<float*>(out),
        proj_w, proj_act, N, d, h, w, Cpad);
  else { set_error("depth_to_space: bad dtype"); return S3D_ERR_INVALID; }
  S3D_LAUNCH_CHECK();
  return S3D_OK;
}

__global__ void split_tf32_kernel(const float4* __restrict__ x, float4* __restrict__ hi, float4* __restrict__ lo, int64_t n4) {
  for (int64_t i = blockIdx.x * (int64_t)blockDim.x + threadIdx.x; i < n4; i += (int64_t)gridDim.x * blockDim.x) {
    const float4 v = __ldg(x + i);
    float4 h, l;
    h.x = __uint_as_float(__float_as_uint(v.x) & 0xFFFFE000u);  l.x = v.x - h.x;
    h.y = __uint_as_float(__float_as_uint(v.y) & 0xFFFFE000u);  l.y = v.y - h.y;
    h.z = __uint_as_float(__float_as_uint(v.z) & 0xFFFFE000u);  l.z = v.z - h.z;
    h.w = __uint_as_float(__float_as_uint(v.w) & 0xFFFFE000u);  l.w = v.w - h.w;
    hi[i] = h;  lo[i] = l;
  }
}

extern "C" int s3d_split_tf32(const float* x, float* hi, float* lo, int64_t n, void* stream) {
  if (!x || !hi || !lo) { set_error("split_tf32: null argument"); return S3D_ERR_INVALID; }
  S3D_CHECK_ARG(n > 0 && n % 4 == 0, "split_tf32: element count must be a positive multiple of 4");
  S3D_CHECK_ARG(((reinterpret_cast<uintptr_t>(x) | reinterpret_cast<uintptr_t>(hi) | reinterpret_cast<uintptr_t>(lo)) & 15) == 0,
                "split_tf32: pointers must be 16-byte aligned");
  split_tf32_kernel<<<grid_for(n / 4, 256), 256, 0, static_cast<cudaStream_t>(stream)>>>(
      reinterpret_cast<const float4*>(x), reinterpret_cast<float4*>(hi), reinterpret_cast<float4*>(lo), n / 4);
  S3D_LAUNCH_CHECK();
  return S3D_OK;
}

__global__ void unsplit_kernel(const __nv_bfloat16* __restrict__ x, float* __restrict__ out, int64_t npix, int C) {
  const int64_t total = npix * C;
  for (int64_t i = blockIdx.x * (int64_t)blockDim.x + threadIdx.x; i < total; i += (int64_t)gridDim.x * blockDim.x) {
    const int64_t pix = i / C;  const int c = (int)(i % C);
    const __nv_bfloat16* q = x + pix * 2 * C + c;
    out[i] = __bfloat162float(q[0]) + __bfloat162float(q[C]);
  }
}
__global__ void split_kernel(const float* __restrict__ x, __nv_bfloat16* __restrict__ out, int64_t npix, int C) {
  const int64_t total = npix * C;
  for (int64_t i = blockIdx.x * (int64_t)blockDim.x + threadIdx.x; i < total; i += (int64_t)gridDim.x * blockDim.x) {
    const int64_t pix = i / C;  const int c = (int)(i % C);
    const float v = x[i];
    const __nv_bfloat16 hi = __float2bfloat16_rn(v);
    __nv_bfloat16* q = out + pix * 2 * C + c;
    q[0] = hi;  q[C] = __float2bfloat16_rn(v - __bfloat162float(hi));
  }
}

extern "C" int s3d_split_bf16(const float* x, void* out, int64_t npix, int C, void* stream) {
  if (!x || !out) { set_error("split_bf16: null argument"); return S3D_ERR_INVALID; }
  S3D_CHECK_ARG(npix > 0 && C > 0, "split_bf16: bad shape");
  split_kernel<<<grid_for(npix * C, 256), 256, 0, static_cast<cudaStream_t>(stream)>>>(x, static_cast<__nv_bfloat16*>(out), npix, C);
  S3D_LAUNCH_CHECK();
  return S3D_OK;
}
extern "C" int s3d_unsplit_bf16(const void* x, float* out, int64_t npix, int C, void* stream) {
  if (!x || !out) { set_error("unsplit_bf16: null argument"); return S3D_ERR_INVALID; }
  S3D_CHECK_ARG(npix > 0 && C > 0, "unsplit_bf16: bad shape");
  unsplit_kernel<<<grid_for(npix * C, 256), 256, 0, static_cast<cudaStream_t>(stream)>>>(static_cast<const __nv_bfloat16*>(x), out, npix, C);
  S3D_LAUNCH_CHECK();
  return S3D_OK;
}

static int pool_launch(const void* x, void* out, int N, int H, int W, int C, int L, int dtype, int to_vox, void* stream) {
  if (!x || !out) { set_error("pool: null argument"); return S3D_ERR_INVALID; }
  S3D_CHECK_ARG(N > 0 && H > 0 && W > 0 && C > 0 && L > 0, "pool: bad shape");
  S3D_CHECK_ARG(!to_vox || (C * L * L) % 8 == 0, "latent_to_vox: C*L*L must be a multiple of 8");
  cudaStream_t st = static_cast<cudaStream_t>(stream);
  const int64_t total = (int64_t)N * L * L * C;
  if (dtype == S3D_DTYPE_BF16X2)
    pool_split_kernel<<<grid_for(total, 256), 256, 0, st>>>(static_cast<const __nv_bfloat16*>(x), static_cast<__nv_bfloat16*>(out), N, H, W, C, L, to_vox);
  else if (dtype == S3D_DTYPE_BF16)
    pool_kernel<__nv_bfloat16><<<grid_for(total, 256), 256, 0, st>>>(static_cast<const __nv_bfloat16*>(x), static_cast<__nv_bfloat16*>(out), N, H, W, C, L, to_vox);
  else if (dtype == S3D_DTYPE_F32)
    pool_kernel<float><<<grid_for(total, 256), 256, 0, st>>>(static_cast<const float*>(x), static_cast<float*>(out), N, H, W, C, L, to_vox);
  else { set_error("pool: bad dtype"); return S3D_ERR_INVALID; }
  S3D_LAUNCH_CHECK();
  return S3D_OK;
}

extern "C" int s3d_latent_to_vox(const void* x, void* out, int N, int H, int W, int C, int L, int dtype, void* stream) {
  return pool_launch(x, out, N, H, W, C, L, dtype, 1, stream);
}
extern "C" int s3d_avg_pool(const void* x, void* out, int N, int H, int W, int C, int L, int dtype, void* stream) {
  return pool_launch(x, out, N, H, W, C, L, dtype, 0, stream);
}

extern "C" int s3d_fuse_views(const void* score, int64_t score_stride, const void* vol, int64_t vol_stride, int dtype,
                              float* fused, int B, int V, int nvox, const uint8_t* gt, const float* thresholds, int T,
                              long long* iou, int64_t score_lo, int64_t vol_lo, void* stream) {
  if (!score || !vol || !fused) { set_error("fuse_views: null argument"); return S3D_ERR_INVALID; }
  S3D_CHECK_ARG(B > 0 && V > 0 && nvox > 0 && T >= 0 && T <= kMaxThresh, "fuse_views: bad shape (T<=8)");
  S3D_CHECK_ARG(!gt || (thresholds && iou), "fuse_views: gt needs thresholds and iou");
  Thresh th;
  for (int t = 0; t < kMaxThresh; ++t) th.t[t] = (gt && t < T) ? thresholds[t] : 2.f;
  cudaStream_t st = static_cast<cudaStream_t>(stream);
  dim3 grid(ceil_div(nvox, 256 * 4), B);
  S3D_CHECK_ARG(dtype == S3D_DTYPE_BF16X2 ? (score_lo > 0 && vol_lo > 0) : (score_lo == 0 && vol_lo == 0),
                "fuse_views: score_lo / vol_lo are the lo-part offsets of split (BF16X2) tensors, 0 otherwise");
  if (dtype == S3D_DTYPE_BF16 || dtype == S3D_DTYPE_BF16X2)
    fuse_views_kernel<__nv_bfloat16><<<grid, 256, 0, st>>>(static_cast<const __nv_bfloat16*>(score), score_stride, static_cast<const __nv_bfloat16*>(vol), vol_stride, fused, B, V, nvox, gt, th, T, reinterpret_cast<unsigned long long*>(iou), score_lo, vol_lo);
  else if (dtype == S3D_DTYPE_F32)
    fuse_views_kernel<float><<<grid, 256, 0, st>>>(static_cast<const float*>(score), score_stride, static_cast<const float*>(vol), vol_stride, fused, B, V, nvox, gt, th, T, reinterpret_cast<unsigned long long*>(iou), 0, 0);
  else { set_error("fuse_views: bad dtype"); return S3D_ERR_INVALID; }
  S3D_LAUNCH_CHECK();
  return S3D_OK;
}
```

### stereo_3d_reconstruction_b200/layers.py

```python
import ctypes
import os
import itertools

import torch

from . import lib as _lib

PAD = 16


def pad_to(c, m=PAD):
    return (c + m - 1) // m * m


def torch_dtype(code):
    return torch.float32 if code == _lib.DTYPE_F32 else torch.bfloat16


def is_split(code):
    return code == _lib.DTYPE_BF16X2


def cmult(code):
    return 2 if code == _lib.DTYPE_BF16X2 else 1


def to_storage(w, code):
    if code == _lib.DTYPE_F32:
        return w.float()
    hi = w.to(torch.bfloat16)
    if code == _lib.DTYPE_BF16:
        return hi
    lo = (w.float() - hi.float()).to(torch.bfloat16)
    return torch.cat([hi, lo], -1)


def from_storage(t, code):
    if code != _lib.DTYPE_BF16X2:
        return t.float()
    c = t.shape[-1] // 2
    return t[..., :c].float() + t[..., c:].float()


def _fold_bn(w_out_first, bias, bn):
    w = w_out_first.detach().float()
    cout = w.shape[0]
    b = bias.detach().float() if bias is not None else torch.zeros(cout, device=w.device)
    if bn is not None:
        scale = bn.weight.detach().float() / torch.sqrt(bn.running_var.detach().float() + bn.eps)
        shift = bn.bias.detach().float() - bn.running_mean.detach().float() * scale
        w = w * scale.view(-1, *([1] * (w.dim() - 1)))
        b = b * scale + shift
    return w, b


def _choose_tile(N, oD, oH, oW, sx, sy, sz):
    best = None
    for lw, lh, ld in itertools.product(range(8), repeat=3):
        ln = 7 - lw - lh - ld
        if ln < 0:
            continue
        tw, th, td, tn = 1 << lw, 1 << lh, 1 << ld, 1 << ln
        if tw * sx > 256 or th * sy > 256 or td * sz > 256:
            continue
        waste = (-(-oW // tw) * tw) * (-(-oH // th) * th) * (-(-oD // td) * td) * (-(-N // tn) * tn)
        key = (waste, -lw, -lh, -ld)
        if best is None or key < best[0]:
            best = (key, (tw, th, td, tn))
    return best[1]


def _choose_bn(cout_pad, m_tiles=None, n_sms=148):
    divs = [bn for bn in range(min(256, cout_pad), 15, -16) if cout_pad % bn == 0]
    if not divs:
        raise ValueError('no N tile for Cout=%d' % cout_pad)
    if m_tiles is None:
        return divs[0]
    for bn in divs:
        if m_tiles * (cout_pad // bn) >= n_sms * 3 // 4:
            return bn
    return divs[-1]


class PackedConv:

    def __init__(self, w_rows, bias, taps, stride, out_mult, cin, cout, act, act_param, dtype_code, device,
                 ksize=(1, 1, 1), pad=(0, 0, 0)):
        self._ctor = (w_rows.detach().float().cpu(), bias.detach().float().cpu(), taps, stride, out_mult, cin,
                      cout, act, act_param, dtype_code, device, tuple(ksize), tuple(pad))
        self.n_classes = len(taps)
        self.ntaps = len(taps[0])
        assert self.n_classes * self.ntaps <= _lib.S3D_MAX_TAPS
        self.cin, self.cout = cin, cout
        self.cin_pad, self.cout_pad = pad_to(cin), pad_to(cout)
        self.stride = stride
        self.out_mult = out_mult
        self.act, self.act_param = act, float(act_param)
        self.dtype_code = dtype_code
        wp = torch.zeros(self.n_classes * self.ntaps, self.cout_pad, self.cin_pad, dtype=torch.float32)
        wp[:, :cout, :cin] = w_rows.cpu()
        self.weight = to_storage(wp, dtype_code).to(device).contiguous()
        bp = torch.zeros(self.cout_pad, dtype=torch.float32)
        bp[:cout] = bias.cpu()
        self.bias = bp.to(device)
        self.taps = taps
        self.ksize, self.pad = tuple(ksize), tuple(pad)
        self.weight_ns = None
        if tuple(ksize) == (3, 3, 3) and tuple(pad) == (1, 1, 1) and tuple(stride) == (1, 1, 1) and \
                self.n_classes == 1 and self.cout_pad <= 64:
            w3 = wp.view(3, 9, self.cout_pad, self.cin_pad)
            self.weight_ns = to_storage(self.pack_nstack(w3), dtype_code).to(device).contiguous()
        self.bn = _choose_bn(self.cout_pad)
        self.proj = None
        self._cache = {}
        self.vol = None
        row_bytes = self.cin_pad * (4 if dtype_code == _lib.DTYPE_F32 else 2) * cmult(dtype_code)
        if tuple(ksize) == (1, 3, 3) and tuple(pad) == (0, 1, 1) and tuple(stride) == (1, 1, 1) and \
                self.n_classes == 1 and self.cout_pad <= 64 and \
                row_bytes in ((64, 128, 256) if is_split(dtype_code) else (32, 64, 128)) and \
                (not is_split(dtype_code) or self.cout_pad in (16, 32, 64)) and \
                [tuple(t) for t in taps[0]] == [(0, dy, dx) for dy in (-1, 0, 1) for dx in (-1, 0, 1)]:
            w27 = torch.zeros(27, cout, cin, dtype=torch.float32)
            w27[9:18] = w_rows.cpu()
            taps27 = [[(dz, dy, dx) for dz in (-1, 0, 1) for dy in (-1, 0, 1) for dx in (-1, 0, 1)]]
            self.vol = PackedConv(w27, bias, taps27, (1, 1, 1), (1, 1, 1), cin, cout, act, act_param, dtype_code, device,
                                  ksize=(3, 3, 3), pad=(1, 1, 1))

    def derive(self, w_rows, bias, act):
        _, _, taps, stride, out_mult, cin, cout, _, act_param, dtype_code, device, ksize, pad = self._ctor
        pc = PackedConv(w_rows, bias, taps, stride, out_mult, cin, cout, act, act_param, dtype_code, device, ksize=ksize, pad=pad)
        for k in ('ntaps_algo', 'block_cout'):
            if hasattr(self, k):
                setattr(pc, k, getattr(self, k))
        return pc

    @staticmethod
    def pack_nstack(w3):
        _, _, co, ci = w3.shape
        ns = torch.zeros(4, 9, 3 * co, ci, dtype=torch.float32)
        for r in range(4):
            for s in range(3):
                if r == 3 and s == 2:
                    continue
                ns[r, :, s * co:(s + 1) * co] = w3[((r % 3) + 1 - s) % 3]
        return ns.view(36, 3 * co, ci)

    def refonce_weights(self, C):
        key = ('refonce', C)
        if key not in self._cache:
            assert self.ntaps == 27 and self.n_classes == 1 and self.cin_pad == 2 * C
            w3 = self._ctor[0].view(3, 9, self.cout, self.cin)
            ro = torch.zeros(3, 9, self.cout_pad, C, dtype=torch.float32)
            cr = min(C, self.cin)
            ro[0, :, :self.cout, :cr] = w3[:, :, :, :cr].sum(0)
            ro[1, :, :self.cout, :cr] = -w3[0, :, :, :cr]
            ro[2, :, :self.cout, :cr] = -w3[2, :, :, :cr]
            self._cache[key] = to_storage(ro.view(27, self.cout_pad, C), self.dtype_code).to(self.weight.device).contiguous()
        return self._cache[key]

    def gonce_convs(self, C, pad, w, D):
        key = ('gonce', C, pad, w, D)
        if key in self._cache:
            return self._cache[key]
        assert self.ntaps == 27 and self.n_classes == 1 and self.cin == 2 * C and self.dtype_code in (_lib.DTYPE_BF16, _lib.DTYPE_BF16X2)
        A = self.cout
        Ap = self.cout_pad
        W = self._ctor[0].view(3, 3, 3, A, 2 * C)
        Wl, Wr = W[..., :C], W[..., C:]
        dev = self.weight.device
        P = w + 2 * pad
        assert pad >= 2 and pad + w - D + 2 <= 127, 'tap offsets are int8'
        out = {}
        es = (-2, -1, 0, 1, 2)
        for name, sgn in (('left', 1), ('right', -1)):
            rows = torch.zeros(15, 6 * Ap, C)
            for iy in range(3):
                for ie, e in enumerate(es):
                    r = rows[iy * 5 + ie]
                    if -1 <= e <= 1:
                        r[0 * Ap:0 * Ap + A] = Wl[:, iy, e + 1].sum(0)
                        r[1 * Ap:1 * Ap + A] = -Wl[0, iy, e + 1]
                        r[2 * Ap:2 * Ap + A] = -Wl[2, iy, e + 1]
                    for kz in range(3):
                        dx = e - sgn * (kz - 1)
                        if -1 <= dx <= 1:
                            r[3 * Ap:3 * Ap + A] += Wr[kz, iy, dx + 1]
                            if kz == 0:
                                r[4 * Ap:4 * Ap + A] -= Wr[kz, iy, dx + 1]
                            if kz == 2:
                                r[5 * Ap:5 * Ap + A] -= Wr[kz, iy, dx + 1]
            taps = [[(0, dy, e + pad - 2) for dy in (-1, 0, 1) for e in es]]
            out[name + '_geom'] = (pad - 4, 5, w + 4)
            out[name] = PackedConv(rows, torch.zeros(6 * Ap), taps, (1, 1, 1), (1, 1, 1), C, 6 * Ap, _lib.ACT_NONE, 0.0,
                                   self.dtype_code, dev, ksize=(1, 3, P - (w + 4) + 1), pad=(0, 1, 0))
            dxe = -1 if name == 'left' else 1
            rows = torch.zeros(9, 4 * Ap, C)
            for iy in range(3):
                for kz in range(3):
                    e = dxe + sgn * (kz - 1)
                    ie = e + 2 if name == 'left' else e
                    r = rows[iy * 3 + ie]
                    r[0:A] -= Wr[kz, iy, dxe + 1]
                    if kz == 0:
                        r[Ap:Ap + A] += Wr[kz, iy, dxe + 1]
                    if kz == 2:
                        r[2 * Ap:2 * Ap + A] += Wr[kz, iy, dxe + 1]
            off = (pad - 2) if name == 'left' else (pad + w - D)
            taps = [[(0, dy, ie + off) for dy in (-1, 0, 1) for ie in range(3)]]
            out['edge_' + name + '_geom'] = (off, 3, D)
            out['edge_' + name] = PackedConv(rows, torch.zeros(4 * Ap), taps, (1, 1, 1), (1, 1, 1), C, 4 * Ap, _lib.ACT_NONE, 0.0,
                                             self.dtype_code, dev, ksize=(1, 3, P - D + 1), pad=(0, 1, 0))
        self._cache[key] = out
        return out

    @classmethod
    def from_conv(cls, conv, bn, act, dtype_code, device, act_param=0.0):
        w, b = _fold_bn(conv.weight, conv.bias, bn)
        if w.dim() == 4:
            w = w.unsqueeze(2)
            ks, st, pd = (1,) + tuple(conv.kernel_size), (1,) + tuple(conv.stride), (0,) + tuple(conv.padding)
        else:
            ks, st, pd = tuple(conv.kernel_size), tuple(conv.stride), tuple(conv.padding)
        cout, cin = w.shape[0], w.shape[1]
        taps, rows = [], []
        for kz, ky, kx in itertools.product(range(ks[0]), range(ks[1]), range(ks[2])):
            taps.append((kz - pd[0], ky - pd[1], kx - pd[2]))
            rows.append(w[:, :, kz, ky, kx])
        return cls(torch.stack(rows), b, [taps], st, (1, 1, 1), cin, cout, act, act_param, dtype_code, device,
                   ksize=ks, pad=pd)

    @classmethod
    def from_deconv_k4s2p1(cls, deconv, bn, act, dtype_code, device, act_param=0.0):
        assert tuple(deconv.kernel_size) == (4, 4, 4) and tuple(deconv.stride) == (2, 2, 2) and \
            tuple(deconv.padding) == (1, 1, 1) and tuple(deconv.output_padding) == (0, 0, 0)
        w, b = _fold_bn(deconv.weight.transpose(0, 1), deconv.bias, bn)
        cout, cin = w.shape[0], w.shape[1]
        per_dim = {0: [(0, 1), (-1, 3)], 1: [(1, 0), (0, 2)]}
        taps, rows = [], []
        for cz, cy, cx in itertools.product(range(2), repeat=3):
            ct = []
            for (oz, kz), (oy, ky), (ox, kx) in itertools.product(per_dim[cz], per_dim[cy], per_dim[cx]):
                ct.append((oz, oy, ox))
                rows.append(w[:, :, kz, ky, kx])
            taps.append(ct)
        return cls(torch.stack(rows), b, taps, (1, 1, 1), (2, 2, 2), cin, cout, act, act_param, dtype_code, device)

    @classmethod
    def from_deconv_k4s2p1_blocked(cls, deconv, bn, act, dtype_code, device, act_param=0.0):
        assert tuple(deconv.kernel_size) == (4, 4, 4) and tuple(deconv.stride) == (2, 2, 2) and \
            tuple(deconv.padding) == (1, 1, 1) and tuple(deconv.output_padding) == (0, 0, 0)
        w, b = _fold_bn(deconv.weight.transpose(0, 1), deconv.bias, bn)
        cout, cin = w.shape[0], w.shape[1]
        kof = {0: {0: 1, -1: 3}, 1: {1: 0, 0: 2}}
        taps, rows = [], []
        for dz, dy, dx in itertools.product((-1, 0, 1), repeat=3):
            m = torch.zeros(8 * cout, cin, dtype=w.dtype)
            for cz, cy, cx in itertools.product(range(2), repeat=3):
                if dz in kof[cz] and dy in kof[cy] and dx in kof[cx]:
                    c = (cz * 2 + cy) * 2 + cx
                    m[c * cout:(c + 1) * cout] = w[:, :, kof[cz][dz], kof[cy][dy], kof[cx][dx]]
            taps.append((dz, dy, dx))
            rows.append(m)
        pc = cls(torch.stack(rows), b.repeat(8), [taps], (1, 1, 1), (1, 1, 1), cin, 8 * cout, act, act_param, dtype_code,
                 device, ksize=(3, 3, 3), pad=(1, 1, 1))
        pc.ntaps_algo = 8
        pc.block_cout = cout
        return pc

    @classmethod
    def from_pointwise(cls, w_out_in, bias, bn, act, dtype_code, device, act_param=0.0):
        w, b = _fold_bn(w_out_in, bias, bn)
        return cls(w.unsqueeze(0), b, [[(0, 0, 0)]], (1, 1, 1), (1, 1, 1), w.shape[1], w.shape[0], act, act_param,
                   dtype_code, device)

    @classmethod
    def from_linear_over_map(cls, linear, C, h, w_, act, dtype_code, device, act_param=0.0):
        w, b = _fold_bn(linear.weight, linear.bias, None)
        w = w.view(w.shape[0], C, h, w_)
        taps, rows = [], []
        for y, x in itertools.product(range(h), range(w_)):
            taps.append((0, y, x))
            rows.append(w[:, :, y, x])
        return cls(torch.stack(rows), b, [taps], (1, 1, 1), (1, 1, 1), C, w.shape[0], act, act_param, dtype_code,
                   device, ksize=(1, h, w_), pad=(0, 0, 0))

    def set_projection(self, w_vec, channel, act):
        assert self.cout_pad == 16 and self.cout <= channel < 16, (self.cout_pad, self.cout, channel)
        v = torch.zeros(16, dtype=torch.float32)
        v[:self.cout] = w_vec.detach().float().cpu().flatten()[:self.cout]
        self.proj = (v.to(self.weight.device), int(channel), int(act))
        self._cache = {}
        return self

    def out_grid(self, iD, iH, iW):
        if self.n_classes == 8:
            return iD, iH, iW
        return tuple((i + 2 * p - k) // s + 1 for i, k, p, s in zip((iD, iH, iW), self.ksize, self.pad, self.stride))

    def params(self, N, iD, iH, iW, out_strides, out_dtype_code, cout_store=None, os_lo=0):
        key = (N, iD, iH, iW, tuple(out_strides), out_dtype_code, cout_store, os_lo)
        p = self._cache.get(key)
        if p is not None:
            return p
        oD, oH, oW = self.out_grid(iD, iH, iW)
        p = _lib.S3dConvParams()
        p.N, p.iD, p.iH, p.iW, p.Cin = N, iD, iH, iW, self.cin_pad
        p.oD, p.oH, p.oW, p.Cout = oD, oH, oW, self.cout_pad
        p.sz, p.sy, p.sx = self.stride
        p.ntaps, p.n_classes = self.ntaps, self.n_classes
        i = 0
        for ct in self.taps:
            for (dz, dy, dx) in ct:
                p.dz[i], p.dy[i], p.dx[i] = dz, dy, dx
                i += 1
        p.osN, p.osD, p.osH, p.osW = out_strides[:4]
        p.osC = out_strides[4] if len(out_strides) > 4 else 1
        p.os_lo = os_lo
        p.omz, p.omy, p.omx = self.out_mult
        p.cout_store = self.cout_pad if cout_store is None else cout_store
        p.in_dtype, p.out_dtype = self.dtype_code, out_dtype_code
        p.act, p.act_param = self.act, self.act_param
        p.tw, p.th, p.td, p.tn = _choose_tile(N, oD, oH, oW, self.stride[2], self.stride[1], self.stride[0])
        m_tiles = self.n_classes * -(-oW // p.tw) * -(-oH // p.th) * -(-oD // p.td) * -(-N // p.tn)
        p.bn = _choose_bn(self.cout_pad, m_tiles)
        p.w_nstack = self.weight_ns.data_ptr() if self.weight_ns is not None else None
        if self.proj is not None:
            p.proj_w, p.proj_channel, p.proj_act = self.proj[0].data_ptr(), self.proj[1], self.proj[2]
        self._cache[key] = p
        return p

    def __call__(self, x, out=None, residual=None, out_dtype=None, cout_store=None, out_view=None, engine='igemm'):
        cm = cmult(self.dtype_code)
        assert x.is_cuda and x.is_contiguous() and x.dim() == 5 and x.shape[-1] == cm * self.cin_pad, \
            (tuple(x.shape), self.cin_pad)
        assert x.dtype == torch_dtype(self.dtype_code)
        N, iD, iH, iW, _ = x.shape
        oD, oH, oW = self.out_grid(iD, iH, iW)
        m = self.out_mult
        odt = x.dtype if out_dtype is None else out_dtype
        if out is None:
            out = torch.empty((N, oD * m[0], oH * m[1], oW * m[2], self.cout_pad * (cm if odt == torch.bfloat16 else 1)),
                              dtype=odt, device=x.device)
        if out.dtype == torch.float32:
            code = _lib.DTYPE_F32
        else:
            code = _lib.DTYPE_BF16X2 if is_split(self.dtype_code) else _lib.DTYPE_BF16
        if self._halo2d_ok(x, out, residual, cout_store, out_view, engine):
            return self._call_halo2d(x, out, residual, out_view)
        if self.vol is not None and engine == 'igemm' and iD == 1 and self.proj is None and \
                (out_view is None or len(out_view[1]) == 4) and (out.dtype == x.dtype or not is_split(self.dtype_code)) and not _lib.KNOBS['no_vol2d'] and not _lib.KNOBS['no_scatter']:
            return self._call_as_volume(x, out, residual, cout_store, out_view)
        if out_view is None:
            assert out.is_contiguous() and out.dim() == 5
            C = out.shape[-1]
            strides = (out.shape[1] * out.shape[2] * out.shape[3] * C, out.shape[2] * out.shape[3] * C,
                       out.shape[3] * C, C)
            off = 0
            if cout_store is None:
                cout_store = min(self.cout_pad, C)
            if code == _lib.DTYPE_BF16X2:
                assert C == 2 * self.cout_pad, 'split output: [.., hi(Cout_pad) | lo(Cout_pad)]'
            os_lo = 0
        else:
            off, strides = out_view[:2]
            os_lo = out_view[2] if len(out_view) > 2 else 0
            assert code != _lib.DTYPE_BF16X2 or os_lo > 0, 'a split output view needs its hi -> lo offset'
        p = self.params(N, iD, iH, iW, strides, code, cout_store, os_lo)
        L = _lib.load()
        fn = L.s3d_conv_igemm if engine == 'igemm' else L.s3d_conv_direct
        esz = out.element_size()
        rptr = None
        if residual is not None:
            assert residual.dtype == out.dtype and residual.shape == out.shape and residual.is_contiguous()
            rptr = residual.data_ptr() + off * esz
        rc = fn(ctypes.byref(p), x.data_ptr(), self.weight.data_ptr(), self.bias.data_ptr(), rptr,
                out.data_ptr() + off * esz, torch.cuda.current_stream().cuda_stream)
        _lib.check(rc, 's3d_conv_%s' % engine)
        _lib.count_launch()
        return out

    def _halo2d_ok(self, x, out, residual, cout_store, out_view, engine):
        return (engine == 'igemm' and x.shape[1] == 1 and self.dtype_code == _lib.DTYPE_BF16 and out.dtype == torch.bfloat16 and
                self.ksize == (1, 3, 3) and self.pad == (0, 1, 1) and tuple(self.stride) == (1, 1, 1) and self.n_classes == 1 and
                self.cin_pad in (32, 64) and self.cout_pad in (32, 64) and
                self.act in (_lib.ACT_NONE, _lib.ACT_RELU) and
                self.proj is None and (cout_store is None or cout_store == self.cout_pad) and
                (out_view is None or (len(out_view[1]) == 4 and (len(out_view) < 3 or not out_view[2]))) and
                [tuple(t) for t in self.taps[0]] == [(0, dy, dx) for dy in (-1, 0, 1) for dx in (-1, 0, 1)] and
                not _lib.KNOBS['no_conv2d_halo'] and not _lib.KNOBS['no_scatter'])

    def _call_halo2d(self, x, out, residual, out_view):
        N, _, H, W, _ = x.shape
        if out_view is None:
            assert out.is_contiguous() and out.dim() == 5 and out.shape[-1] >= self.cout_pad
            Co = out.shape[-1]
            off, sN, sH, sW = 0, out.shape[2] * out.shape[3] * Co, out.shape[3] * Co, Co
        else:
            off, (sN, _, sH, sW) = out_view[:2]
        rptr = None
        if residual is not None:
            assert residual.dtype == out.dtype and residual.shape == out.shape and residual.is_contiguous()
            rptr = residual.data_ptr() + off * 2
        rc = _lib.load().s3d_conv2d_halo(x.data_ptr(), self.weight.data_ptr(), self.bias.data_ptr(), rptr, out.data_ptr() + off * 2,
                                         N, H, W, self.cin_pad, self.cout_pad, sN, sH, sW, int(self.act == _lib.ACT_RELU),
                                         torch.cuda.current_stream().cuda_stream)
        _lib.check(rc, 's3d_conv2d_halo')
        _lib.count_launch()
        return out

    def _call_as_volume(self, x, out, residual, cout_store, out_view):
        N, _, H, W, C = x.shape
        patches = -(-H // 32) * -(-W // 8)
        G = min((g for g in range(1, N + 1) if N % g == 0),
                key=lambda g: (-(-g * patches // 148) * (N // g + 2), g))
        Dv = N // G
        if out_view is None:
            assert out.is_contiguous() and out.dim() == 5
            Co = out.shape[-1]
            sN, sH, sW = out.shape[2] * out.shape[3] * Co, out.shape[3] * Co, Co
            off = 0
            if cout_store is None:
                cout_store = min(self.cout_pad, Co)
            os_lo = self.cout_pad
        else:
            off, (sN, _, sH, sW) = out_view[:2]
            os_lo = out_view[2] if len(out_view) > 2 else 0
        self.vol(x.view(G, Dv, H, W, C), out=out, residual=residual, cout_store=cout_store,
                 out_view=(off, (Dv * sN, sN, sH, sW), os_lo))
        return out

    def flops(self, N, iD, iH, iW):
        oD, oH, oW = self.out_grid(iD, iH, iW)
        return 2.0 * N * oD * oH * oW * self.n_classes * self.cout * self.cin * getattr(self, 'ntaps_algo', self.ntaps)


class SplitConv:

    def __init__(self, pc):
        assert pc.dtype_code == _lib.DTYPE_F32 and pc.proj is None
        w, b = pc._ctor[0], pc._ctor[1]
        w_hi = (w.view(torch.int32) & -8192).view(torch.float32)
        self.full = pc
        self.hi = pc.derive(w_hi, torch.zeros_like(b), _lib.ACT_NONE)
        self.lo = pc.derive(w - w_hi, b, pc.act)
        for k in ('cin', 'cout', 'cin_pad', 'cout_pad', 'ksize', 'stride', 'pad', 'n_classes', 'out_mult', 'act', 'act_param',
                  'dtype_code', 'weight', 'bias', 'proj'):
            setattr(self, k, getattr(pc, k))

    def out_grid(self, *a):
        return self.full.out_grid(*a)

    def flops(self, *a):
        return self.full.flops(*a)

    def __call__(self, x, out=None, residual=None, engine='igemm', **kw):
        from . import ops
        assert engine == 'igemm' and x.dtype == torch.float32
        x_hi, x_lo = ops.split_tf32(x)
        out = self.hi(x_hi, out=out, residual=residual, **kw)
        self.hi(x_lo, out=out, residual=out, **kw)
        self.lo(x_hi, out=out, residual=out, **kw)
        return out
```

### stereo_3d_reconstruction_b200/lib.py

```python
import ctypes
import os

_HERE = os.path.dirname(os.path.abspath(__file__))
LIB_PATH = os.environ.get('S3D_LIB_PATH') or os.path.join(_HERE, 'libs3d_b200.so')

S3D_MAX_TAPS = 64
DTYPE_F32, DTYPE_BF16, DTYPE_BF16X2 = 0, 1, 2
ACT_NONE, ACT_RELU, ACT_LEAKY, ACT_SIGMOID, ACT_TANH = 0, 1, 2, 3, 4


class S3dConvParams(ctypes.Structure):
    _fields_ = [
        ('N', ctypes.c_int32), ('iD', ctypes.c_int32), ('iH', ctypes.c_int32), ('iW', ctypes.c_int32),
        ('Cin', ctypes.c_int32),
        ('oD', ctypes.c_int32), ('oH', ctypes.c_int32), ('oW', ctypes.c_int32), ('Cout', ctypes.c_int32),
        ('sz', ctypes.c_int32), ('sy', ctypes.c_int32), ('sx', ctypes.c_int32),
        ('ntaps', ctypes.c_int32), ('n_classes', ctypes.c_int32),
        ('dz', ctypes.c_int8 * S3D_MAX_TAPS), ('dy', ctypes.c_int8 * S3D_MAX_TAPS),
        ('dx', ctypes.c_int8 * S3D_MAX_TAPS),
        ('osN', ctypes.c_int64), ('osD', ctypes.c_int64), ('osH', ctypes.c_int64), ('osW', ctypes.c_int64),
        ('osC', ctypes.c_int64),
        ('os_lo', ctypes.c_int64),
        ('omz', ctypes.c_int32), ('omy', ctypes.c_int32), ('omx', ctypes.c_int32),
        ('cout_store', ctypes.c_int32),
        ('in_dtype', ctypes.c_int32), ('out_dtype', ctypes.c_int32),
        ('act', ctypes.c_int32), ('act_param', ctypes.c_float),
        ('tw', ctypes.c_int32), ('th', ctypes.c_int32), ('td', ctypes.c_int32), ('tn', ctypes.c_int32),
        ('bn', ctypes.c_int32),
        ('proj_w', ctypes.c_void_p), ('proj_channel', ctypes.c_int32), ('proj_act', ctypes.c_int32),
        ('w_nstack', ctypes.c_void_p),
    ]


_vp, _i, _f, _i64 = ctypes.c_void_p, ctypes.c_int, ctypes.c_float, ctypes.c_int64
_CONV_SIG = [ctypes.POINTER(S3dConvParams), _vp, _vp, _vp, _vp, _vp, _vp]

SIGNATURES = {
    's3d_version': ([], ctypes.c_char_p),
    's3d_last_error': ([], ctypes.c_char_p),
    's3d_device_check': ([_i], _i),
    's3d_set_knob': ([ctypes.c_char_p, _i], _i),
    's3d_get_knob': ([ctypes.c_char_p], _i),
    's3d_conv_igemm': (_CONV_SIG, _i),
    's3d_conv_direct': (_CONV_SIG, _i),
    's3d_pack_image': ([_vp, _vp, _f, _vp, _i, _i, _i, _i, _i, _vp], _i),
    's3d_pack_image_u8': ([_vp, _vp, _f, _f, _vp, _i, _i, _i, _i, _i, _vp], _i),
    's3d_conv_first': ([_vp, _i, _vp, _f, _vp, _vp, _vp, _i, _i, _i, _i, _i, _i, _i, _i, _f, _vp], _i),
    's3d_conv_concat_volume': ([ctypes.POINTER(S3dConvParams), _vp, _i, _i, _vp, _vp, _vp], _i),
    's3d_conv_concat_volume_ro': ([ctypes.POINTER(S3dConvParams), _vp, _i, _i, _vp, _vp, _vp, _vp], _i),
    's3d_conv_cls_workspace_bytes': ([_i, _i, _i, _i], ctypes.c_int64),
    's3d_conv_cls_soft_argmin': ([ctypes.POINTER(S3dConvParams), _vp, _vp, _vp, _vp, _vp, ctypes.c_float, _vp], _i),
    's3d_conv2d_halo': ([_vp, _vp, _vp, _vp, _vp, _i, _i, _i, _i, _i, _i64, _i64, _i64, _i, _vp], _i),
    's3d_map_conv': ([_vp, _vp, _vp, _i, _i, _i, _i, _i, _i, _i, _i, _vp], _i),
    's3d_concat_gonce_assemble': ([_vp, _vp, _vp, _vp, _vp, _vp, _i, _i, _i, _i, _i, _i, _vp], _i),
    's3d_cost_volume_concat': ([_vp, _vp, _i, _i, _i, _i, _i, _i, _vp], _i),
    's3d_soft_argmin': ([_vp, _vp, _i, _i, _i, _i, _f, _vp], _i),
    's3d_tap_gather_soft_argmin': ([_vp, _vp, _vp, _i, _i, _i, _i, _i, _f, _vp], _i),
    's3d_cls_soft_argmin': ([_vp, _vp, _vp, _i, _i, _i, _i, _i, _f, _vp], _i),
    's3d_corr_soft_argmin': ([_vp, _vp, _vp, _i, _i, _i, _i, _i, _i, _i, _vp], _i),
    's3d_upsample_disp': ([_vp, _vp, _i, _i, _i, _i, _i, _f, _vp], _i),
    's3d_upsample_disp_eval': ([_vp, _vp, _vp, ctypes.POINTER(_f), _i, _f, _vp, _i, _i, _i, _i, _i, _f, _vp], _i),
    's3d_upsample_disp_lr': ([_vp, _vp, _vp, _f, _vp, ctypes.POINTER(_f), _i, _f, _vp, _vp, _i, _i, _i, _i, _i, _f, _vp], _i),
    's3d_latent_to_vox': ([_vp, _vp, _i, _i, _i, _i, _i, _i, _vp], _i),
    's3d_avg_pool': ([_vp, _vp, _i, _i, _i, _i, _i, _i, _vp], _i),
    's3d_depth_to_space': ([_vp, _vp, _vp, _i, _i, _i, _i, _i, _i, _i, _vp], _i),
    's3d_split_tf32': ([_vp, _vp, _vp, _i64, _vp], _i),
    's3d_split_bf16': ([_vp, _vp, _i64, _i, _vp], _i),
    's3d_unsplit_bf16': ([_vp, _vp, _i64, _i, _vp], _i),
    's3d_fuse_views': ([_vp, _i64, _vp, _i64, _i, _vp, _i, _i, _i, _vp, ctypes.POINTER(_f), _i, _vp, _i64, _i64, _vp], _i),
    's3d_chamfer_forward': ([_vp, _vp, _vp, _vp, _vp, _vp, _i, _i, _i, _vp], _i),
    's3d_chamfer_workspace_bytes': ([_i, _i, _i], ctypes.c_int64),
    's3d_chamfer_forward_ws': ([_vp, _vp, _vp, _vp, _vp, _vp, _i, _i, _i, _vp, _i64, _vp], _i),
    's3d_chamfer_eval': ([_vp, _vp, _vp, _vp, _vp, _vp, _i, _i, _i, ctypes.POINTER(_f), _i, _vp, _vp, _i64, _vp], _i),
    's3d_fma_probe': ([_vp, _i, ctypes.POINTER(ctypes.c_int64), _vp], _i),
}

_lib = None


class S3dError(RuntimeError):
    pass


def load():
    global _lib
    if _lib is not None:
        return _lib
    if not os.path.exists(LIB_PATH):
        raise S3dError(
            'libs3d_b200.so not found at %s -- build it with `python -c "import __graft_entry__ as g; g.build()"` '
            '(or `make -C stereo_3d_reconstruction_b200/csrc`).  There is no CPU fallback.' % LIB_PATH)
    lib = ctypes.CDLL(LIB_PATH)
    for name, (argtypes, restype) in SIGNATURES.items():
        fn = getattr(lib, name)
        fn.argtypes = argtypes
        fn.restype = restype
    _lib = lib
    return lib


def check(rc, what):
    if rc != 0:
        msg = load().s3d_last_error().decode('utf-8', 'replace')
        raise S3dError('%s failed (rc=%d): %s' % (what, rc, msg))


HOST_KNOBS = ('no_vol2d', 'no_concat_fuse', 'no_cls_fused', 'no_conv_first', 'no_d2s', 'no_ref_once', 'no_cls_chain', 'no_sheared', 'no_map_conv', 'no_conv2d_halo')
LIB_KNOBS = ('no_scatter', 'scatter_tps3', 'scatter_no_pair', 'scatter_ring', 'scatter_res_transpose',
             'scatter_no_transpose', 'scatter_generic', 'no_corr_tc', 'scatter_zsplit', 'scatter_no_rm', 'igemm_ts1', 'igemm_one_cta', 'scatter_one_cta', 'no_conv_first_tc', 'chamfer_sym', 'chamfer_sym_r')
KNOBS = {k: int(os.environ.get('S3D_' + k.upper()) is not None) for k in HOST_KNOBS}
KNOBS['no_scatter'] = int(os.environ.get('S3D_NO_SCATTER') is not None)


def set_knob(name, value):
    value = int(value)
    if name in LIB_KNOBS:
        check(load().s3d_set_knob(name.encode(), value), 's3d_set_knob')
    elif name not in HOST_KNOBS:
        raise KeyError('unknown knob %r' % name)
    if name in KNOBS:
        KNOBS[name] = value


_launches = 0


def count_launch(n=1):
    global _launches
    _launches += n


def launches():
    return _launches
```

### stereo_3d_reconstruction_b200/models.py

```python
import math
import os

import torch
import torch.nn as nn

from . import lib as _lib
from . import ops
from .layers import PackedConv, SplitConv, pad_to, torch_dtype, cmult

A = _lib

PRECISIONS = ('bf16', 'bf16x3', 'tf32', 'tf32x3', 'fp32')


def _conv_bn2d(cin, cout, k, s, p):
    return nn.Sequential(nn.Conv2d(cin, cout, k, s, p, bias=False), nn.BatchNorm2d(cout))


def _conv_bn3d(cin, cout):
    return nn.Sequential(nn.Conv3d(cin, cout, 3, 1, 1, bias=False), nn.BatchNorm3d(cout))


class _FeatureEncoder(nn.Module):
    def __init__(self, cfg):
        super().__init__()
        c1, c2 = cfg.NETWORK.ENC_CHANNELS
        cf = cfg.NETWORK.FEAT_CHANNELS
        self.conv0 = _conv_bn2d(3, c1, 3, 2, 1)
        self.conv1 = _conv_bn2d(c1, c1, 3, 1, 1)
        self.conv2 = _conv_bn2d(c1, c2, 3, 2, 1)
        self.conv3 = _conv_bn2d(c2, c2, 3, 1, 1)
        self.conv4 = _conv_bn2d(c2, c2, 3, 1, 1)
        self.conv5 = nn.Conv2d(c2, cf, 3, 1, 1, bias=True)


class _CostAggregation(nn.Module):
    def __init__(self, cfg):
        super().__init__()
        cin, a = 2 * cfg.NETWORK.FEAT_CHANNELS, cfg.NETWORK.AGG_CHANNELS
        self.dres0a = _conv_bn3d(cin, a)
        self.dres0b = _conv_bn3d(a, a)
        self.dres1a = _conv_bn3d(a, a)
        self.dres1b = _conv_bn3d(a, a)
        self.cls_a = _conv_bn3d(a, a)
        self.cls_b = nn.Conv3d(a, 1, 3, 1, 1, bias=False)


class _DispNet(nn.Module):
    def __init__(self, cfg):
        super().__init__()
        self.encoder = _FeatureEncoder(cfg)
        if cfg.NETWORK.COST_VOLUME == 'concat':
            self.aggregation = _CostAggregation(cfg)


class _RGBDEncoder(nn.Module):
    def __init__(self, cfg):
        super().__init__()
        ch = [4] + list(cfg.NETWORK.REC_CHANNELS)
        self.layers = nn.ModuleList([_conv_bn2d(ch[i], ch[i + 1], 3, 2, 1) for i in range(len(ch) - 1)])


class _VoxelDecoder(nn.Module):
    def __init__(self, cfg):
        super().__init__()
        ch = list(cfg.NETWORK.DEC_CHANNELS)
        self.layers = nn.ModuleList([
            nn.Sequential(nn.ConvTranspose3d(ch[i], ch[i + 1], 4, 2, 1, bias=False), nn.BatchNorm3d(ch[i + 1]))
            for i in range(len(ch) - 1)])
        self.out = nn.ConvTranspose3d(ch[-1], 1, 1, bias=False)


class _Merger(nn.Module):
    def __init__(self, cfg):
        super().__init__()
        ch = list(cfg.NETWORK.MERGER_CHANNELS)
        self.layers = nn.ModuleList([_conv_bn3d(ch[i], ch[i + 1]) for i in range(len(ch) - 1)])


class _PointDecoder(nn.Module):
    def __init__(self, cfg):
        super().__init__()
        c, L = cfg.NETWORK.REC_CHANNELS[-1], cfg.NETWORK.LATENT_HW
        self.conv = _conv_bn2d(2 * c, 2 * c, 3, 2, 1)
        self.fc1 = nn.Linear(2 * c * (L // 2) * (L // 2), cfg.NETWORK.POINT_FC)
        self.fc2 = nn.Linear(cfg.NETWORK.POINT_FC, cfg.CONST.N_POINTS * 3)


def init_synthetic_weights(model, seed=0):
    g = torch.Generator().manual_seed(seed + 12345)
    gains = {'decoder.out': 3.0, 'merger.layers.4.0': 4.0, 'point_decoder.fc2': 2.0}
    with torch.no_grad():
        for name, m in model.named_modules():
            if isinstance(m, (nn.Conv2d, nn.Conv3d, nn.Linear, nn.ConvTranspose3d)):
                w = m.weight
                if isinstance(m, nn.ConvTranspose3d):
                    taps = 1
                    for k, s in zip(m.kernel_size, m.stride):
                        taps *= max(k // s, 1)
                    fan_in = w.shape[0] * taps
                else:
                    fan_in = w[0].numel()
                std = (2.0 / fan_in) ** 0.5 * gains.get(name, 1.0)
                w.copy_((torch.randn(w.shape, generator=g) * std).to(w.device))
                if m.bias is not None:
                    m.bias.copy_((torch.randn(m.bias.shape, generator=g) * 0.1).to(w.device))
            elif isinstance(m, (nn.BatchNorm2d, nn.BatchNorm3d)):
                n, dev = m.num_features, m.weight.device
                m.running_mean.copy_((torch.randn(n, generator=g) * 0.1).to(dev))
                m.running_var.copy_((torch.rand(n, generator=g) + 0.5).to(dev))
                m.weight.copy_((torch.rand(n, generator=g) * 0.4 + 0.8).to(dev))
                m.bias.copy_((torch.randn(n, generator=g) * 0.1).to(dev))
    return model.eval()


class _GraphedForward:

    def __init__(self, model, left, right, gt, disp_gt=None, lr_check=False):
        self.left, self.right = torch.empty_like(left), torch.empty_like(right)
        self.gt = None if gt is None else torch.empty_like(gt)
        self.disp_gt = None if disp_gt is None else torch.empty_like(disp_gt)
        self._copy_in(left, right, gt, disp_gt)
        args = (self.left, self.right) if gt is None else (self.left, self.right, self.gt)
        kw = {} if disp_gt is None else {'disp_gt': self.disp_gt}
        if lr_check:
            kw['lr_check'] = True

        def run():
            return model._forward_impl(*args, **kw)
        side = torch.cuda.Stream(device=left.device)
        side.wait_stream(torch.cuda.current_stream())
        with torch.cuda.stream(side):
            for _ in range(2):
                run()
        torch.cuda.current_stream().wait_stream(side)
        self.graph = torch.cuda.CUDAGraph()
        with torch.cuda.graph(self.graph):
            self.out = run()

    def _copy_in(self, left, right, gt, disp_gt):
        self.left.copy_(left, non_blocking=True)
        self.right.copy_(right, non_blocking=True)
        if self.gt is not None:
            self.gt.copy_(gt, non_blocking=True)
        if self.disp_gt is not None:
            self.disp_gt.copy_(disp_gt, non_blocking=True)

    def __call__(self, left, right, gt, disp_gt=None):
        self._copy_in(left, right, gt, disp_gt)
        self.graph.replay()
        return self.out


class _StereoBase(nn.Module):

    def __init__(self, cfg):
        super().__init__()
        self.cfg = cfg
        self.dispnet = _DispNet(cfg)
        self.rgbd_encoder = _RGBDEncoder(cfg)
        self._packed = None
        self._ws = {}
        self._graphs = {}
        self._packed_prec = None
        self.register_load_state_dict_post_hook(lambda module, incompatible: module._invalidate())

    def _invalidate(self):
        self._packed = None
        self._ws = {}
        self._graphs = {}

    def _apply(self, fn, *args, **kwargs):
        r = super()._apply(fn, *args, **kwargs)
        self._invalidate()
        return r

    def train(self, mode=True):
        self._invalidate()
        return super().train(mode)

    @property
    def precision(self):
        return self.cfg.NETWORK.PRECISION

    def _dtype_code(self):
        if self.precision not in PRECISIONS:
            raise ValueError('NETWORK.PRECISION must be one of %s, got %r' % (PRECISIONS, self.precision))
        return {'bf16': A.DTYPE_BF16, 'bf16x3': A.DTYPE_BF16X2}.get(self.precision, A.DTYPE_F32)

    @property
    def _split(self):
        return self.precision == 'bf16x3'

    def _engine(self):
        return 'direct' if self.precision == 'fp32' else 'igemm'

    def pack(self):
        cfgn = self.cfg.NETWORK
        if cfgn.DEC_CHANNELS[0] % 16 or cfgn.REC_CHANNELS[-1] % 16:
            raise ValueError('NETWORK.DEC_CHANNELS[0] and NETWORK.REC_CHANNELS[-1] must be multiples of 16')
        dev = next(self.parameters()).device
        if dev.type != 'cuda':
            raise _lib.S3dError('Stereo2Voxel/Stereo2Point run on CUDA only (no CPU fallback); call .cuda() first')
        _lib.load()
        dc = self._dtype_code()
        P = {}
        e = self.dispnet.encoder
        for i in range(5):
            seq = getattr(e, 'conv%d' % i)
            P['enc%d' % i] = PackedConv.from_conv(seq[0], seq[1], A.ACT_NONE if i == 4 else A.ACT_RELU, dc, dev)
        P['enc5'] = PackedConv.from_conv(e.conv5, None, A.ACT_NONE, dc, dev)
        if self.cfg.NETWORK.COST_VOLUME == 'concat':
            ag = self.dispnet.aggregation
            for n in ('dres0a', 'dres0b', 'dres1a', 'dres1b', 'cls_a'):
                seq = getattr(ag, n)
                P[n] = PackedConv.from_conv(seq[0], seq[1], A.ACT_NONE if n == 'dres1b' else A.ACT_RELU, dc, dev)
            wb = ag.cls_b.weight
            P['cls_b'] = PackedConv.from_pointwise(wb[0].reshape(wb.shape[1], 27).t(), None, None, A.ACT_NONE, dc, dev)
        for i, seq in enumerate(self.rgbd_encoder.layers):
            P['rec%d' % i] = PackedConv.from_conv(seq[0], seq[1], A.ACT_RELU, dc, dev)
        self._pack_head(P, dc, dev)
        if self.precision == 'tf32x3':
            P = {k: SplitConv(v) for k, v in P.items()}
        self._packed = P
        self._packed_prec = self.precision
        self._ws = {}
        self._graphs = {}
        return self

    def _pack_head(self, P, dc, dev):
        raise NotImplementedError

    def _buf(self, name, shape, dtype, zero=False):
        key = (name, tuple(shape), dtype)
        t = self._ws.get(key)
        if t is None:
            dev = next(self.parameters()).device
            t = (torch.zeros if zero else torch.empty)(shape, dtype=dtype, device=dev)
            self._ws[key] = t
        return t

    def _conv(self, name, x, **kw):
        return self._packed[name](x, engine=self._engine(), **kw)

    @staticmethod
    def _bhw(img):
        return (img.shape[0], img.shape[1], img.shape[2]) if img.dtype == torch.uint8 else (img.shape[0], img.shape[2], img.shape[3])

    def _disparity(self, left, right, disp_gt=None, lr_check=False):
        cfg = self.cfg
        B, H, W = self._bhw(left)
        D = cfg.NETWORK.MAX_DISP
        dt = torch_dtype(self._dtype_code())
        x = self._first('enc0', 'e0', 'img', left, right, None, 1.0)
        x = self._conv('enc1', x, out=self._bufo('e1', 'enc1', x))
        x = self._conv('enc2', x, out=self._bufo('e2', 'enc2', x))
        y = self._conv('enc3', x, out=self._bufo('e3', 'enc3', x))
        x = self._conv('enc4', y, residual=x, out=self._bufo('e4', 'enc4', y))
        h, w = x.shape[2], x.shape[3]
        C = cfg.NETWORK.FEAT_CHANNELS
        p5, p0 = self._packed['enc5'], self._packed.get('dres0a')
        ro_split = (self._split and C == 32 and isinstance(p0, PackedConv) and p0.cout_pad == 64 and p0.act == _lib.ACT_RELU and
                    not _lib.KNOBS['no_ref_once'])
        sheared = (cfg.NETWORK.COST_VOLUME == 'concat' and (self.precision == 'bf16' or ro_split) and C == 32 and p5.cout_pad == C and
                   isinstance(p0, PackedConv) and p0.weight_ns is not None and p0.cout_pad == 64 and p0.act == _lib.ACT_RELU and
                   D >= 4 and w + 2 <= 127 and not _lib.KNOBS['no_sheared'] and not _lib.KNOBS['no_concat_fuse'] and
                   not _lib.KNOBS['no_scatter'])
        fuse_volume = (cfg.NETWORK.COST_VOLUME == 'concat' and (self.precision in ('bf16', 'tf32') or ro_split) and p5.cout_pad == C and
                       isinstance(p0, PackedConv) and p0.weight_ns is not None and
                       (ro_split or C * x.element_size() in (32, 64)) and
                       not _lib.KNOBS['no_concat_fuse'] and not _lib.KNOBS['no_scatter'] and
                       (sheared or 2 * B * (-(-h // 32)) * (-(-w // 8)) > 74))
        cm = cmult(self._dtype_code())
        if fuse_volume:
            pad, P = D, w + 2 * D
            Cp = cm * C
            featp = self._buf('featp', (2 * B, 1, h, P, Cp), dt, zero=True)
            self._conv('enc5', x, out=featp, out_view=(pad * Cp, (h * P * Cp, h * P * Cp, P * Cp, Cp), C if self._split else 0),
                       cout_store=C)
            feat = None
        else:
            feat = self._conv('enc5', x, out=self._bufo('e5', 'enc5', x))
        disp_q = self._buf('disp_q', (2 * B, h, w), torch.float32)
        if cfg.NETWORK.COST_VOLUME == 'concat':
            if fuse_volume:
                ro = ro_split or (self.precision == 'bf16' and p0.cout_pad == 64 and p0.act == _lib.ACT_RELU and
                                  not _lib.KNOBS['no_ref_once'])
                if sheared:
                    bufs = {'maps_l': self._buf('sh_ml', (B, 1, h, w + 4, 384), torch.float32),
                            'maps_r': self._buf('sh_mr', (B, 1, h, w + 4, 384), torch.float32),
                            'edge_l': self._buf('sh_el', (B, 1, h, D, 256), torch.float32),
                            'edge_r': self._buf('sh_er', (B, 1, h, D, 256), torch.float32)}
                    a = ops.conv_concat_volume_sheared(p0, featp, B, D, pad, out=self._buf('a0', (2 * B, D, h, w, cm * 64), dt), bufs=bufs)
                else:
                    a = ops.conv_concat_volume(p0, featp, B, D, pad, out=self._buf('a0', (2 * B, D, h, w, cm * p0.cout_pad), dt),
                                               ref_once=ro)
            else:
                assert feat.shape[-1] == cm * C, 'FEAT_CHANNELS must be a multiple of 16'
                vol = ops.cost_volume_concat(feat, B, D, out=self._buf('vol', (2 * B, D, h, w, 2 * cm * C), dt), split=self._split)
                a = self._conv('dres0a', vol, out=self._bufo('a0', 'dres0a', vol))
            a = self._conv('dres0b', a, out=self._bufo('a1', 'dres0b', a))
            y = self._conv('dres1a', a, out=self._bufo('a2', 'dres1a', a))
            a = self._conv('dres1b', y, residual=a, out=self._bufo('a3', 'dres1b', y))
            S = self._packed['cls_b'].cout_pad
            pa = self._packed['cls_a']
            if (self.precision == 'bf16' and isinstance(pa, PackedConv) and pa.weight_ns is not None and pa.cin_pad == 64 and
                    pa.cout_pad == 64 and pa.act == _lib.ACT_RELU and S == 32 and a.shape[-1] == 64 and
                    2 * B * (-(-h // 32)) * (-(-w // 8)) > 74 and
                    not _lib.KNOBS['no_cls_chain'] and not _lib.KNOBS['no_cls_fused'] and not _lib.KNOBS['no_scatter']):
                nb = ops.conv_cls_workspace_bytes(2 * B, D, h, w)
                ops.conv_cls_soft_argmin(pa, a, self._packed['cls_b'].weight, -1.0, out=disp_q,
                                         workspace=self._buf('cls_ws', (nb,), torch.uint8))
                disp, stats, lr = self._upsample_disp(disp_q, H, W, disp_gt, lr_check)
                return disp, disp_q, stats, lr
            c = self._conv('cls_a', a, out=self._bufo('a0', 'cls_a', a))
            if self.precision == 'bf16' and c.shape[-1] in (16, 32, 64) and S == 32 and not _lib.KNOBS['no_cls_fused']:
                ops.cls_soft_argmin(c, self._packed['cls_b'].weight, -1.0, out=disp_q)
            else:
                taps = self._buf('taps', (2 * B, D, h, S, w), torch.float32)
                self._conv('cls_b', c, out=taps, out_view=(0, (D * h * S * w, h * S * w, S * w, 1, w)), cout_store=S)
                ops.tap_gather_soft_argmin(taps, -1.0, out=disp_q)
        else:
            if self._split:
                feat = ops.unsplit_bf16(feat, out=self._buf('feat32', feat.shape[:-1] + (feat.shape[-1] // 2,), torch.float32))
            ops.corr_soft_argmin(feat, B, D, out=disp_q, c_real=C)
        disp, stats, lr = self._upsample_disp(disp_q, H, W, disp_gt, lr_check)
        return disp, disp_q, stats, lr

    def _upsample_disp(self, disp_q, H, W, disp_gt, lr_check=False):
        B = disp_q.shape[0] // 2
        out = self._buf('disp', (2 * B, H, W), torch.float32)
        th = list(self.cfg.TEST.DISP_THRESH)
        stats = None
        if disp_gt is not None:
            stats = self._buf('disp_stats', (B, 2, 2 + len(th)), torch.int64)
            stats.zero_()
        max_gt = 4.0 * self.cfg.NETWORK.MAX_DISP
        if lr_check:
            tau = float(self.cfg.TEST.LR_THRESH)
            if not (math.isfinite(tau) and tau >= 0):
                raise ValueError('TEST.LR_THRESH must be finite and >= 0, got %r' % self.cfg.TEST.LR_THRESH)
            mask = self._buf('lr_mask', (B, 2, H, W), torch.uint8)
            lr_stats = self._buf('lr_stats', (B, 2, 3 + len(th)), torch.int64)
            lr_stats.zero_()
            ops.upsample_disp_lr(disp_q, H, W, 4.0, tau, mask, lr_stats, gt=disp_gt, thresholds=th, max_gt=max_gt, stats=stats,
                                 out=out)
            return out, stats, (mask, lr_stats)
        if disp_gt is None:
            return ops.upsample_disp(disp_q, H, W, 4.0, out=out), None, None
        ops.upsample_disp_eval(disp_q, H, W, 4.0, disp_gt, th, max_gt, stats, out=out)
        return out, stats, None

    def _bufo(self, name, layer, x):
        pc = self._packed[layer]
        N, iD, iH, iW, _ = x.shape
        oD, oH, oW = pc.out_grid(iD, iH, iW)
        m = pc.out_mult
        return self._buf(name, (N, oD * m[0], oH * m[1], oW * m[2], pc.cout_pad * cmult(pc.dtype_code)), x.dtype)

    def _latent(self, left, right, disp):
        B, H, W = self._bhw(left)
        dt = torch_dtype(self._dtype_code())
        scale = 1.0 / (4.0 * self.cfg.NETWORK.MAX_DISP)
        x = self._first('rec0', 'r0', 'rgbd', left, right, disp, scale)
        for i in range(1, len(self.rgbd_encoder.layers)):
            x = self._conv('rec%d' % i, x, out=self._bufo('r%d' % i, 'rec%d' % i, x))
        return x

    def _first(self, layer, out_name, stage_name, left, right, disp, scale):
        B, H, W = self._bhw(left)
        pc = self._packed[layer]
        dt = torch_dtype(self._dtype_code())
        if pc.ksize == (1, 3, 3) and pc.stride == (1, 2, 2) and pc.pad == (0, 1, 1) and pc.cout_pad in (16, 32, 64) and \
                not _lib.KNOBS['no_conv_first']:
            oH, oW = (H - 1) // 2 + 1, (W - 1) // 2 + 1
            out = self._buf(out_name, (2 * B, 1, oH, oW, pc.cout_pad * cmult(pc.dtype_code)), dt)
            ops.conv_first(left, pc, None if disp is None else disp[:B], scale, out=out[:B])
            ops.conv_first(right, pc, None if disp is None else disp[B:], scale, out=out[B:])
            return out
        if self._split:
            raise _lib.S3dError("'bf16x3' needs the direct first layer (3x3 stride-2 conv, <= 64 output channels)")
        x = self._buf(stage_name, (2 * B, 1, H, W, 16), dt)
        ops.pack_image(left, None if disp is None else disp[:B], scale, out=x[:B])
        ops.pack_image(right, None if disp is None else disp[B:], scale, out=x[B:])
        return self._conv(layer, x, out=self._bufo(out_name, layer, x))

    def graphed(self, left, right, gt=None, *, disp_gt=None, lr_check=False):
        left, right = self._check_inputs(left, right)
        gt = self._check_gt(gt, left)
        disp_gt = self._check_disp_gt(disp_gt, left)
        mb = int(self.cfg.CONST.get('MICRO_BATCH', 0) or 0)
        if mb and left.shape[0] > mb:
            raise ValueError('graphed(): batch %d exceeds CONST.MICRO_BATCH = %d; use forward()' % (left.shape[0], mb))
        key = (tuple(left.shape), left.dtype, None if gt is None else (tuple(gt.shape), gt.dtype),
               None if disp_gt is None else (tuple(disp_gt.shape), disp_gt.dtype), bool(lr_check))
        g = self._graphs.get(key)
        if g is None:
            g = _GraphedForward(self, left, right, gt, disp_gt, bool(lr_check))
            self._graphs[key] = g
        return g(left, right, gt, disp_gt)

    def _check_inputs(self, left, right):
        if self._packed is None or self._packed_prec != self.precision:
            self.pack()
        if not (left.is_cuda and right.is_cuda):
            raise _lib.S3dError('inputs must be CUDA tensors (no CPU fallback)')
        if left.dtype == torch.uint8 and right.dtype == torch.uint8:
            if left.shape != right.shape or left.dim() != 4 or left.shape[3] != 3:
                raise ValueError('expected uint8 left/right of shape [B,H,W,3], got %s / %s' % (tuple(left.shape), tuple(right.shape)))
            return left.contiguous(), right.contiguous()
        if left.shape != right.shape or left.dim() != 4 or left.shape[1] != 3:
            raise ValueError('expected left/right of shape [B,3,H,W], got %s / %s' % (tuple(left.shape), tuple(right.shape)))
        return left.contiguous().float(), right.contiguous().float()

    def _check_gt(self, gt, left):
        return gt

    def _check_disp_gt(self, disp_gt, left):
        if disp_gt is None:
            return None
        B, H, W = self._bhw(left)
        if not isinstance(disp_gt, torch.Tensor):
            raise ValueError('disp_gt must be a tensor, got %s' % type(disp_gt).__name__)
        if tuple(disp_gt.shape) != (B, 2, H, W):
            raise ValueError('expected disp_gt of shape %s, got %s' % ((B, 2, H, W), tuple(disp_gt.shape)))
        if disp_gt.dtype != torch.float32:
            raise ValueError('disp_gt must be float32, got %s' % disp_gt.dtype)
        if disp_gt.device != left.device:
            raise ValueError('disp_gt must be on %s (the images\' device), got %s' % (left.device, disp_gt.device))
        return disp_gt.contiguous()


class Stereo2Voxel(_StereoBase):

    def __init__(self, cfg):
        super().__init__(cfg)
        self.decoder = _VoxelDecoder(cfg)
        self.merger = _Merger(cfg)
        assert cfg.NETWORK.MERGER_CHANNELS[0] == cfg.NETWORK.DEC_CHANNELS[-1] + 1

    def _pack_head(self, P, dc, dev):
        for i, seq in enumerate(self.decoder.layers):
            P['dec%d' % i] = PackedConv.from_deconv_k4s2p1(seq[0], seq[1], A.ACT_RELU, dc, dev)
        w = self.decoder.out.weight
        nl = len(self.decoder.layers)
        last = P['dec%d' % (nl - 1)]
        self._d2s = None
        self._fused_out = False
        row_bytes = last.cin_pad * (4 if dc == A.DTYPE_F32 else 2) * cmult(dc)
        seq = self.decoder.layers[nl - 1]
        if last.cout == 8 and row_bytes in ((64, 128, 256) if self._split else (32, 64, 128)) and self.precision != 'fp32' and \
                not _lib.KNOBS['no_d2s']:
            P['dec%d' % (nl - 1)] = PackedConv.from_deconv_k4s2p1_blocked(seq[0], seq[1], A.ACT_RELU, dc, dev)
            pw = torch.zeros(8, dtype=torch.float32)
            pw[:] = w.detach().float().cpu().view(-1)[:8]
            self._d2s = pw.to(dev)
            self._fused_out = True
        elif self._split:
            raise _lib.S3dError("'bf16x3' needs DEC_CHANNELS[-1] == 8 and DEC_CHANNELS[-2] in (16, 32, 64) (blocked last deconv)")
        elif last.cout_pad == 16 and last.cout < 16 and self.precision != 'tf32x3':
            self._fused_out = True
            last.set_projection(w.view(-1), last.cout, A.ACT_SIGMOID)
        else:
            P['dec_out'] = PackedConv.from_pointwise(w.view(w.shape[0], 1).t(), None, None, A.ACT_SIGMOID, dc, dev)
        for i, seq in enumerate(self.merger.layers):
            P['mrg%d' % i] = PackedConv.from_conv(seq[0], seq[1], A.ACT_LEAKY, dc, dev,
                                                  act_param=self.cfg.NETWORK.LEAKY_VALUE)

    def forward(self, left, right, gt=None, *, disp_gt=None, lr_check=False):
        left, right = self._check_inputs(left, right)
        disp_gt = self._check_disp_gt(disp_gt, left)
        mb = int(self.cfg.CONST.get('MICRO_BATCH', 0) or 0)
        B = left.shape[0]
        if mb and B > mb:
            outs = []
            for s in range(0, B, mb):
                o = self._forward_chunk(left[s:s + mb], right[s:s + mb], None if gt is None else gt[s:s + mb],
                                        None if disp_gt is None else disp_gt[s:s + mb], lr_check)
                outs.append(tuple(t.clone() for t in o))
            return tuple(torch.cat(ts, 0) for ts in zip(*outs))
        return self._forward_chunk(left, right, gt, disp_gt, lr_check)

    def _forward_impl(self, left, right, gt=None, disp_gt=None, lr_check=False):
        return self._forward_chunk(left, right, gt, disp_gt, lr_check)

    def _forward_chunk(self, left, right, gt, disp_gt=None, lr_check=False):
        cfg = self.cfg
        B, H, W = self._bhw(left)
        nv = cfg.CONST.N_VOX
        disp, _, dstats, lr = self._disparity(left, right, disp_gt, lr_check)
        x = self._latent(left, right, disp)
        L = cfg.NETWORK.LATENT_HW
        k0 = cfg.NETWORK.DEC_CHANNELS[0]
        km = cmult(self._dtype_code())
        assert x.shape[-1] // km * L * L == k0 * 8, 'REC_CHANNELS[-1]*LATENT_HW^2 must equal DEC_CHANNELS[0]*8'
        x = ops.latent_to_vox(x, L, out=self._buf('lat', (2 * B, 2, 2, 2, km * pad_to(k0)), x.dtype, zero=True), split=self._split)
        nl = len(self.decoder.layers)
        for i in range(nl):
            x = self._conv('dec%d' % i, x, out=self._bufo('d%d' % i, 'dec%d' % i, x))
        if self._d2s is not None:
            n2, dd, hh, ww, _ = x.shape
            x = ops.depth_to_space(x, 16, self._d2s, A.ACT_SIGMOID, split=self._split,
                                   out=self._buf('d2s', (n2, 2 * dd, 2 * hh, 2 * ww, 16 * km), x.dtype))
        m_in = x
        split_lo = m_in.shape[-1] // 2 if self._split else 0
        cm = m_in.shape[-1]
        craw = cfg.NETWORK.DEC_CHANNELS[-1]
        assert m_in.shape[1] == nv and cm > craw
        if not self._fused_out:
            self._conv('dec_out', m_in, out=m_in, out_view=(craw, (nv ** 3 * cm, nv * nv * cm, nv * cm, cm)), cout_store=1)
        s = m_in
        for i in range(len(self.merger.layers)):
            s = self._conv('mrg%d' % i, s, out=self._bufo('m%d' % (i % 2), 'mrg%d' % i, s))
        fused = self._buf('fused', (B, nv ** 3), torch.float32)
        iou = None
        gt8 = None
        if gt is not None:
            th = list(cfg.TEST.VOXEL_THRESH)
            iou = self._buf('iou', (B, len(th), 2), torch.int64)
            iou.zero_()
            gt8 = gt.reshape(B, -1).to(torch.uint8).contiguous()
        ops.fuse_views(s, 0, s.shape[-1], m_in, craw, cm, B, 2, nv ** 3, gt=gt8,
                       thresholds=list(cfg.TEST.VOXEL_THRESH) if gt is not None else None, iou=iou, out=fused,
                       score_lo=s.shape[-1] // 2 if self._split else 0, vol_lo=split_lo)
        out = (disp[:B].unsqueeze(1), disp[B:].unsqueeze(1), fused.view(B, nv, nv, nv))
        if gt is not None:
            out += (iou,)
        if disp_gt is not None:
            out += (dstats,)
        return out + lr if lr_check else out


def fscore_thresholds(cfg):
    th = cfg.TEST.get('FSCORE_THRESH')
    try:
        th = [float(t) for t in th]
    except (TypeError, ValueError):
        raise ValueError('TEST.FSCORE_THRESH must be a list of numbers, got %r' % (th,)) from None
    if len(th) > 8 or not all(math.isfinite(t) and t > 0 for t in th):
        raise ValueError('TEST.FSCORE_THRESH must hold at most 8 finite distances > 0, got %r' % (cfg.TEST.FSCORE_THRESH,))
    return th


class Stereo2Point(_StereoBase):

    def __init__(self, cfg):
        super().__init__(cfg)
        self.point_decoder = _PointDecoder(cfg)

    def _check_gt(self, gt, left):
        if gt is None:
            return None
        B = left.shape[0]
        if not isinstance(gt, torch.Tensor):
            raise ValueError('gt must be a tensor, got %s' % type(gt).__name__)
        if gt.dim() != 3 or gt.shape[0] != B or gt.shape[1] < 1 or gt.shape[2] != 3:
            raise ValueError('expected gt of shape [%d, M, 3], got %s' % (B, tuple(gt.shape)))
        if gt.dtype != torch.float32:
            raise ValueError('gt must be float32, got %s' % gt.dtype)
        if gt.device != left.device:
            raise ValueError('gt must be on %s (the images\' device), got %s' % (left.device, gt.device))
        fscore_thresholds(self.cfg)
        return gt.contiguous()

    def _pack_head(self, P, dc, dev):
        pd = self.point_decoder
        c, L = self.cfg.NETWORK.REC_CHANNELS[-1], self.cfg.NETWORK.LATENT_HW
        P['pt_conv'] = PackedConv.from_conv(pd.conv[0], pd.conv[1], A.ACT_RELU, dc, dev)
        P['pt_fc1'] = PackedConv.from_linear_over_map(pd.fc1, 2 * c, L // 2, L // 2, A.ACT_RELU, dc, dev)
        P['pt_fc2'] = PackedConv.from_pointwise(pd.fc2.weight, pd.fc2.bias, None, A.ACT_TANH, dc, dev, act_param=0.5)

    def forward(self, left, right, gt=None, *, disp_gt=None, lr_check=False):
        left, right = self._check_inputs(left, right)
        return self._forward_impl(left, right, self._check_gt(gt, left), disp_gt=self._check_disp_gt(disp_gt, left),
                                  lr_check=lr_check)

    def _forward_impl(self, left, right, gt=None, disp_gt=None, lr_check=False):
        cfg = self.cfg
        B = left.shape[0]
        disp, _, dstats, lr = self._disparity(left, right, disp_gt, lr_check)
        x = self._latent(left, right, disp)
        L = cfg.NETWORK.LATENT_HW
        if x.shape[2] != L or x.shape[3] != L:
            x = ops.avg_pool(x, L, out=self._buf('pool', (2 * B, 1, L, L, x.shape[-1]), x.dtype), split=self._split)
        c = x.shape[-1]
        cat = self._buf('latcat', (B, 1, L, L, 2 * c), x.dtype)
        if self._split:
            h = c // 2
            cat[..., :h].copy_(x[:B, ..., :h]);  cat[..., h:c].copy_(x[B:, ..., :h])
            cat[..., c:c + h].copy_(x[:B, ..., h:]);  cat[..., c + h:].copy_(x[B:, ..., h:])
        else:
            cat[..., :c].copy_(x[:B])
            cat[..., c:].copy_(x[B:])
        y = self._conv('pt_conv', cat, out=self._bufo('p0', 'pt_conv', cat))
        y = self._conv('pt_fc1', y, out=self._bufo('p1', 'pt_fc1', y))
        npts = cfg.CONST.N_POINTS
        pts = self._buf('pts', (B, 1, 1, 1, pad_to(npts * 3)), torch.float32)
        self._conv('pt_fc2', y, out=pts)
        points = pts.view(B, -1)[:, :npts * 3].reshape(B, npts, 3)
        out = (disp[:B].unsqueeze(1), disp[B:].unsqueeze(1), points)
        if gt is not None:
            out += (self._point_stats(points, gt),)
        if disp_gt is not None:
            out += (dstats,)
        return out + lr if lr_check else out

    def _point_stats(self, points, gt):
        th = fscore_thresholds(self.cfg)
        B, N, M = points.shape[0], points.shape[1], gt.shape[1]
        if not points.is_contiguous():
            points = self._buf('pts_xyz', (B, N, 3), torch.float32).copy_(points)
        stats = self._buf('point_stats', (B, 2, 3 + len(th)), torch.int64)
        stats.zero_()
        nb = ops.chamfer_workspace_bytes(B, N, M)
        ops.chamfer_eval(points, gt, th, stats, workspace=self._buf('cd_ws', (nb,), torch.uint8) if nb else None,
                         out=(self._buf('cd_d1', (B, N), torch.float32), self._buf('cd_d2', (B, M), torch.float32),
                              self._buf('cd_i1', (B, N), torch.int32), self._buf('cd_i2', (B, M), torch.int32)))
        return stats


def build_model(name, cfg, seed=None):
    m = {'Stereo2Voxel': Stereo2Voxel, 'Stereo2Point': Stereo2Point}[name](cfg)
    if seed is not None:
        init_synthetic_weights(m, seed)
    return m.eval()
```

Baseline: 4964.

## Skip recomputing constant disparity planes in 3D conv and replicate stores

In the concat cost volume, planes past a column-dependent disparity threshold are identical, because the shifted right feature falls entirely in the padding. The scatter conv now computes only the first of these constant planes per column, jumps over the rest in multiples of three, and writes the computed result to all skipped planes. A host-built, cost-balanced schedule pairs columns with similar start planes and spreads them across CTA pairs to keep load even. This reduces MMA work and input loads for dres0b, dres1a and dres1b, at the cost of extra host scheduling, replicated stores and reliance on the constant-region assumption being exact.

```diff
diff --git a/include/s3d.h b/include/s3d.h
--- a/include/s3d.h
+++ b/include/s3d.h
@@ -42,6 +42,9 @@
   const float* proj_w;
   int32_t proj_channel, proj_act;
   const void* w_nstack;
+  int32_t dz_nref, dz_c, dz_e, dz_pairs;
+  const int32_t* dz_sched;
+  long long* dz_planes;
 } S3dConvParams;
 
 const char* s3d_version(void);
diff --git a/stereo_3d_reconstruction_b200/csrc/common.cuh b/stereo_3d_reconstruction_b200/csrc/common.cuh
--- a/stereo_3d_reconstruction_b200/csrc/common.cuh
+++ b/stereo_3d_reconstruction_b200/csrc/common.cuh
@@ -47,6 +47,7 @@
   int chamfer_sym;
   int chamfer_sym_r;
   int scatter_no_rm;
+  int no_dz_skip;
 };
 Knobs& knobs();
 
diff --git a/stereo_3d_reconstruction_b200/csrc/conv_scatter.cu b/stereo_3d_reconstruction_b200/csrc/conv_scatter.cu
--- a/stereo_3d_reconstruction_b200/csrc/conv_scatter.cu
+++ b/stereo_3d_reconstruction_b200/csrc/conv_scatter.cu
@@ -80,6 +80,14 @@
     grid -= grid % 2;
     a.ncols_max = (int)((total + grid - 1) / grid);
   } else if ((int64_t)grid > total) grid = (int)total;
+  const bool dz = p.dz_nref > 0 && !tf32 && !split && a.nz == 1 && !knobs().no_dz_skip;
+  if (dz) S3D_CHECK_ARG(p.N == 2 * p.dz_nref && p.dz_c >= 0 && p.dz_e >= 0, "scatter: constant-region descriptor");
+  if (!dz) a.p.dz_nref = 0;
+  if (!dz || !a.pair) a.p.dz_sched = nullptr;
+  if (a.p.dz_sched) {
+    S3D_CHECK_ARG(p.dz_pairs >= 1, "scatter: dz_pairs");
+    grid = 2 * p.dz_pairs;
+  }
   const int w_rows = a.pair ? 3 * a.cp / 2 : 3 * a.cp;
   a.w_tx = a.tps * w_rows * a.row_bytes;
   a.w_bytes = (a.w_tx + 1023) / 1024 * 1024;
diff --git a/stereo_3d_reconstruction_b200/csrc/conv_scatter.cuh b/stereo_3d_reconstruction_b200/csrc/conv_scatter.cuh
--- a/stereo_3d_reconstruction_b200/csrc/conv_scatter.cuh
+++ b/stereo_3d_reconstruction_b200/csrc/conv_scatter.cuh
@@ -75,8 +75,39 @@
 }
 
 __device__ __forceinline__ int cta_cols(const ScArgs& a) {
+  if (a.p.dz_sched) return __ldg(a.p.dz_sched + (blockIdx.x >> 1) + 1) - __ldg(a.p.dz_sched + (blockIdx.x >> 1));
   return a.pair ? a.ncols_max : (a.total_cols - (int)blockIdx.x + (int)gridDim.x - 1) / (int)gridDim.x;
 }
+
+struct Item { Col c; int zs, J; };
+
+__device__ __forceinline__ int dz_first(const ScArgs& a, const Col& c) {
+  if (c.n >= a.p.N) return 0;
+  const int xr = c.n < a.p.dz_nref ? min(c.x0 + kTX - 1, a.p.oW - 1) : a.p.oW - 1 - c.x0;
+  return xr + a.p.dz_c + 2;
+}
+
+__device__ __forceinline__ Item cta_item(const ScArgs& a, int ci) {
+  int mine, other;
+  if (a.p.dz_sched) {
+    const int r = blockIdx.x & 1;
+    const int32_t* e = a.p.dz_sched + a.p.dz_pairs + 1 + 2 * (__ldg(a.p.dz_sched + (blockIdx.x >> 1)) + ci);
+    mine = __ldg(e + r);  other = __ldg(e + (r ^ 1));
+  } else {
+    mine = blockIdx.x + ci * gridDim.x;  other = a.pair ? (mine ^ 1) : mine;
+  }
+  Item it;
+  it.c = decode_col(a, mine);
+  it.zs = 0;  it.J = 0;
+  if (a.p.dz_nref > 0) {
+    const int zs = max(dz_first(a, it.c), dz_first(a, decode_col(a, other))), ze = a.p.oD - 2 - a.p.dz_e;
+    it.zs = zs;
+    it.J = ze - zs >= 3 ? (ze - zs) / 3 * 3 : 0;
+  }
+  return it;
+}
+
+__device__ __forceinline__ int next_plane(const Item& it, int p) { return p == it.zs + 1 ? p + 1 + it.J : p + 1; }
 
 __device__ __forceinline__ uint64_t desc_hi(uint32_t sbo, int row_bytes) {
   const uint64_t layout = row_bytes == 128 ? 2ull : (row_bytes == 64 ? 4ull : 6ull);
@@ -100,7 +131,9 @@
   int ws = 0;  uint32_t wphase = 0;
   int pslot = 0;  uint32_t pphase = 0;
   int pci = 0, pj = 0, issued = 0;
-  Col pc = decode_col(a, blockIdx.x);
+  Item pit{};
+  if (ncols > 0) pit = cta_item(a, 0);
+  const Col& pc = pit.c;
   auto issue_plane = [&](bool blocking) -> bool {
     if (pci >= ncols) return false;
     const uint32_t be = bar_pe + 8 * pslot, bf = bar_pf + 8 * pslot;
@@ -122,9 +155,10 @@
     __syncwarp();
     ++issued;
     if (++pslot == ring) { pslot = 0; pphase ^= 1; }
-    if (++pj == D) {
+    pj = next_plane(pit, pj);
+    if (pj >= D) {
       pj = 0;  ++pci;
-      if (pci < ncols) pc = decode_col(a, blockIdx.x + pci * gridDim.x);
+      if (pci < ncols) pit = cta_item(a, pci);
     }
     return true;
   };
@@ -146,9 +180,10 @@
   };
   for (int ci = 0; ci < ncols; ++ci) {
     int rot = 3;
-    [[maybe_unused]] const Col rc = decode_col(a, blockIdx.x + ci * gridDim.x);
+    const Item it = cta_item(a, ci);
+    [[maybe_unused]] const Col& rc = it.c;
     if constexpr (kRM) load_res(rc, 0);
-    for (int p = 0; p < D; ++p, ++gp) {
+    for (int p = 0; p < D; p = next_plane(it, p), ++gp) {
       while (issued <= gp) issue_plane(true);
       const int ahead = gp + ring;
 #pragma unroll
@@ -169,9 +204,13 @@
         __syncwarp();
         if (++ws == w_stages) { ws = 0; wphase ^= 1; }
       }
-      if constexpr (kRM) { if (p + 1 < D) load_res(rc, p + 1); }
+      if constexpr (kRM) { const int pn = next_plane(it, p); if (pn < D) load_res(rc, pn); }
       rot = (p == 0) ? 1 : (rot == 2 ? 0 : rot + 1);
     }
+  }
+  if (a.p.dz_planes) {
+    if (ptx::elect_one()) atomicAdd(reinterpret_cast<unsigned long long*>(a.p.dz_planes), (unsigned long long)issued);
+    __syncwarp();
   }
 }
 
@@ -183,6 +222,7 @@
   uint32_t rb16, tap_step, tile_off, chunk_step;
   uint32_t idesc;
   int D, ncols;
+  const ScArgs* args = nullptr;
 };
 
 template <bool kPair>
@@ -262,7 +302,8 @@
   const uint32_t x_lo0 = desc_lo(z.planes_u32), x_lo_step = z.slot_bytes >> 4;
   const uint32_t d0 = z.tmem_base, d1 = z.tmem_base + kTP;
   for (int ci = 0; ci < z.ncols; ++ci) {
-    for (int p = 0; p < z.D; ++p) {
+    const Item it = cta_item(*z.args, ci);
+    for (int p = 0; p < z.D; p = next_plane(it, p)) {
       ptx::mbar_wait_u32(z.bar_pf + 8 * pw, pwphase);
       const uint64_t xd0 = z.x_hi | (x_lo0 + pw * x_lo_step);
       const uint64_t xd1 = xd0 + z.tile_off;
@@ -357,7 +398,8 @@
 
 template <int CP, typename TOut, bool kRes, int kAct>
 __device__ __forceinline__ void sc_fast_store(const ScEpi& e, int64_t grp_off, int lane, uint32_t okmask,
-                                              const uint32_t (&v)[CP / 16][16], uint4 (&r)[CP * sizeof(TOut) / 16]) {
+                                              const uint32_t (&v)[CP / 16][16], uint4 (&r)[CP * sizeof(TOut) / 16],
+                                              int ncopy = 0, int64_t zstep = 0) {
   constexpr int NCH = CP * sizeof(TOut) / 16;
   constexpr int CPC = 16 / sizeof(TOut);
   uint4 c[NCH];
@@ -408,20 +450,23 @@
   chunk_transpose<NCH>(c, lane);
   const int j = lane & (NCH - 1);
   TOut* o = reinterpret_cast<TOut*>(e.out) + grp_off + j * CPC;
-#pragma unroll
-  for (int k = 0; k < NCH; ++k)
-    if ((okmask >> k) & 1u) *reinterpret_cast<uint4*>(o + k * e.osW) = c[k];
+  for (int i = 0; i <= ncopy; ++i, o += zstep) {
+#pragma unroll
+    for (int k = 0; k < NCH; ++k)
+      if ((okmask >> k) & 1u) *reinterpret_cast<uint4*>(o + k * e.osW) = c[k];
+  }
 }
 
 template <int CP, typename TOut>
 __device__ __forceinline__ void sc_fast_plane(const ScEpi& e, int64_t grp_off, int lane, uint32_t okmask,
-                                              const uint32_t (&v)[CP / 16][16], uint4 (&r)[CP * sizeof(TOut) / 16]) {
+                                              const uint32_t (&v)[CP / 16][16], uint4 (&r)[CP * sizeof(TOut) / 16],
+                                              int ncopy, int64_t zstep) {
   if (e.slope == 0.f) {
-    if (e.residual) sc_fast_store<CP, TOut, true, 0>(e, grp_off, lane, okmask, v, r);
-    else            sc_fast_store<CP, TOut, false, 0>(e, grp_off, lane, okmask, v, r);
+    if (e.residual) sc_fast_store<CP, TOut, true, 0>(e, grp_off, lane, okmask, v, r, ncopy, zstep);
+    else            sc_fast_store<CP, TOut, false, 0>(e, grp_off, lane, okmask, v, r, ncopy, zstep);
   } else {
-    if (e.residual) sc_fast_store<CP, TOut, true, 2>(e, grp_off, lane, okmask, v, r);
-    else            sc_fast_store<CP, TOut, false, 2>(e, grp_off, lane, okmask, v, r);
+    if (e.residual) sc_fast_store<CP, TOut, true, 2>(e, grp_off, lane, okmask, v, r, ncopy, zstep);
+    else            sc_fast_store<CP, TOut, false, 2>(e, grp_off, lane, okmask, v, r, ncopy, zstep);
   }
 }
 
@@ -441,7 +486,8 @@
   uint32_t aphase = 0;
   const int ncols = cta_cols(a);
   for (int ci = 0; ci < ncols; ++ci) {
-    const Col c = decode_col(a, blockIdx.x + ci * gridDim.x);
+    const Item it = cta_item(a, ci);
+    const Col& c = it.c;
     const bool rowok = c.y0 + yl < a.p.oH && c.n < a.p.N;
     const bool ok = rowok && c.x0 + xl < a.p.oW;
     const int64_t row_off = (int64_t)c.n * a.p.osN + (int64_t)(c.y0 + yl) * a.p.osH + (int64_t)c.x0 * a.p.osW;
@@ -451,7 +497,7 @@
 #pragma unroll
     for (int k = 0; k < NCH; ++k) okmask |= (rowok && c.x0 + xb + k < a.p.oW) ? (1u << k) : 0u;
     int slot = 0, z = 0;
-    for (int p = 0; p < D; ++p) {
+    for (int p = 0; p < D; p = next_plane(it, p)) {
       const int ndrain = (p >= 1 ? 1 : 0) + (p == D - 1 ? 1 : 0);
       uint4 r[NCH];
       if constexpr (kFast) {
@@ -483,16 +529,20 @@
         const int64_t zo = (int64_t)(c.zb + z) * a.p.osD;
         const bool stz = z >= zs0 && z < zs1 && c.zb + z < a.p.oD;
         const uint32_t om = stz ? okmask : 0u;
+        const int ncopy = z == it.zs ? it.J : 0;
         if constexpr (kFast) {
           if (i == 1 && a.residual) sc_res_load<NCH, TOut>(fe, grp_off + zo, fe.osW, lane, om, r);
-          if constexpr (kSRes >= 0) sc_fast_store<CP, TOut, kSRes != 0, kSAct>(fe, grp_off + zo, lane, om, v, r);
-          else sc_fast_plane<CP, TOut>(fe, grp_off + zo, lane, om, v, r);
+          if constexpr (kSRes >= 0) sc_fast_store<CP, TOut, kSRes != 0, kSAct>(fe, grp_off + zo, lane, om, v, r, ncopy, a.p.osD);
+          else sc_fast_plane<CP, TOut>(fe, grp_off + zo, lane, om, v, r, ncopy, a.p.osD);
         } else {
           if (ok && stz) {
-#pragma unroll
-            for (int j = 0; j < CP / 16; ++j) epilogue_store16(ep, pix_off + zo, 16 * j, v[j]);
+            for (int k = 0; k <= ncopy; ++k) {
+#pragma unroll
+              for (int j = 0; j < CP / 16; ++j) epilogue_store16(ep, pix_off + zo + k * a.p.osD, 16 * j, v[j]);
+            }
           }
         }
+        z += ncopy;
         ++z;
         if (++slot == 3) slot = 0;
       }
@@ -702,7 +752,7 @@
                         ptx::smem_u32(&ctrl.w_empty[0]), ptx::smem_u32(&ctrl.acc_full[0]), ptx::smem_u32(&ctrl.acc_empty[0]),
                         desc_hi(kHX * rb, rb), desc_hi(8 * rb, rb), a.slot_bytes, a.w_bytes, a.w_stages, a.ring,
                         (uint32_t)(rb >> 4), (uint32_t)(((kPair ? 3 * a.cp / 2 : 3 * a.cp) * rb) >> 4), (uint32_t)((kTileY * kHX * rb) >> 4), (uint32_t)(a.chunk_stride >> 4), a.idesc,
-                        a.dl, cta_cols(a)};
+                        a.dl, cta_cols(a), &a};
     if constexpr (kSplit) {
       if constexpr (RB == 256) sc_issue<false, 1, 4, kPair, 2, true>(zi);
       else if constexpr (RB == 128) sc_issue<false, 1, 2, kPair, 1, true>(zi);
diff --git a/stereo_3d_reconstruction_b200/csrc/conv_scatter_rm.cu b/stereo_3d_reconstruction_b200/csrc/conv_scatter_rm.cu
--- a/stereo_3d_reconstruction_b200/csrc/conv_scatter_rm.cu
+++ b/stereo_3d_reconstruction_b200/csrc/conv_scatter_rm.cu
@@ -57,7 +57,7 @@
                         ptx::smem_u32(&ctrl.w_empty[0]), ptx::smem_u32(&ctrl.acc_full[0]), ptx::smem_u32(&ctrl.acc_empty[0]),
                         desc_hi(kHX * rb, rb), desc_hi(8 * rb, rb), a.slot_bytes, a.w_bytes, a.w_stages, a.ring,
                         (uint32_t)(rb >> 4), (uint32_t)(((3 * a.cp / 2) * rb) >> 4), (uint32_t)((kTileY * kHX * rb) >> 4),
-                        (uint32_t)(a.chunk_stride >> 4), a.idesc, a.dl, cta_cols(a)};
+                        (uint32_t)(a.chunk_stride >> 4), a.idesc, a.dl, cta_cols(a), &a};
     sc_issue<false, 1, 4, kPair, 1, false, true>(zi, &rs);
   } else if (warp >= 4) {
     sc_epilogue<CP, __nv_bfloat16, true, 0, kSAct>(a, ctrl, tmem_base, warp, lane);
diff --git a/stereo_3d_reconstruction_b200/csrc/voxel.cu b/stereo_3d_reconstruction_b200/csrc/voxel.cu
--- a/stereo_3d_reconstruction_b200/csrc/voxel.cu
+++ b/stereo_3d_reconstruction_b200/csrc/voxel.cu
@@ -38,6 +38,7 @@
     {"igemm_one_cta", "S3D_IGEMM_ONE_CTA", &Knobs::igemm_one_cta},
     {"chamfer_sym", "S3D_CHAMFER_SYM", &Knobs::chamfer_sym},
     {"chamfer_sym_r", "S3D_CHAMFER_SYM_R", &Knobs::chamfer_sym_r},
+    {"no_dz_skip", "S3D_NO_DZ_SKIP", &Knobs::no_dz_skip},
 };
 }
 
diff --git a/stereo_3d_reconstruction_b200/layers.py b/stereo_3d_reconstruction_b200/layers.py
--- a/stereo_3d_reconstruction_b200/layers.py
+++ b/stereo_3d_reconstruction_b200/layers.py
@@ -80,6 +80,51 @@
         if m_tiles * (cout_pad // bn) >= n_sms * 3 // 4:
             return bn
     return divs[-1]
+
+
+
+plane_counter = None
+
+
+def dz_first(col, N, nref, oH, oW, c):
+    cy, cx = -(-oH // 32), -(-oW // 8)
+    if col >= N * cy * cx:
+        return 0
+    n, x0 = col // (cy * cx), (col % cx) * 8
+    xr = min(x0 + 7, oW - 1) if n < nref else oW - 1 - x0
+    return xr + c + 2
+
+
+def dz_jump(zs, D, e):
+    ze = D - 2 - e
+    return (ze - zs) // 3 * 3 if ze - zs >= 3 else 0
+
+
+def dz_march(zs, J, D):
+    out, p = [], 0
+    while p < D:
+        out.append(p)
+        p = p + 1 + J if p == zs + 1 else p + 1
+    return out
+
+
+def dz_schedule(N, nref, oH, oW, D, c, e, npairs):
+    total = N * -(-oH // 32) * -(-oW // 8)
+    first = [dz_first(k, N, nref, oH, oW, c) for k in range(total)]
+    cols = sorted(range(total), key=lambda k: (first[k], k))
+    items = [(cols[i], cols[i + 1] if i + 1 < total else total) for i in range(0, total, 2)]
+    cost = [D - dz_jump(max(first[a], first[b] if b < total else 0), D, e) for a, b in items]
+    load, lists = [0] * npairs, [[] for _ in range(npairs)]
+    for i in sorted(range(len(items)), key=lambda i: (-cost[i], i)):
+        q = min(range(npairs), key=lambda q: (load[q], q))
+        load[q] += cost[i]
+        lists[q].append(items[i])
+    offs, ent = [0], []
+    for lst in lists:
+        offs.append(offs[-1] + len(lst))
+        for a, b in lst:
+            ent += [a, b]
+    return offs + ent, load
 
 
 class PackedConv:
@@ -297,8 +342,8 @@
             return iD, iH, iW
         return tuple((i + 2 * p - k) // s + 1 for i, k, p, s in zip((iD, iH, iW), self.ksize, self.pad, self.stride))
 
-    def params(self, N, iD, iH, iW, out_strides, out_dtype_code, cout_store=None, os_lo=0):
-        key = (N, iD, iH, iW, tuple(out_strides), out_dtype_code, cout_store, os_lo)
+    def params(self, N, iD, iH, iW, out_strides, out_dtype_code, cout_store=None, os_lo=0, region=None):
+        key = (N, iD, iH, iW, tuple(out_strides), out_dtype_code, cout_store, os_lo, region)
         p = self._cache.get(key)
         if p is not None:
             return p
@@ -326,10 +371,18 @@
         p.w_nstack = self.weight_ns.data_ptr() if self.weight_ns is not None else None
         if self.proj is not None:
             p.proj_w, p.proj_channel, p.proj_act = self.proj[0].data_ptr(), self.proj[1], self.proj[2]
+        if region is not None:
+            p.dz_nref, p.dz_c, p.dz_e = region
+            dev = self.weight.device
+            ncols = N * -(-oH // 32) * -(-oW // 8)
+            p.dz_pairs = max(1, min(torch.cuda.get_device_properties(dev).multi_processor_count // 2, -(-ncols // 2)))
+            table, _ = dz_schedule(N, p.dz_nref, oH, oW, oD, p.dz_c, p.dz_e, p.dz_pairs)
+            sched = torch.tensor(table, dtype=torch.int32).to(dev)
+            p.dz_sched, p.dz_sched_keep = sched.data_ptr(), sched
         self._cache[key] = p
         return p
 
-    def __call__(self, x, out=None, residual=None, out_dtype=None, cout_store=None, out_view=None, engine='igemm'):
+    def __call__(self, x, out=None, residual=None, out_dtype=None, cout_store=None, out_view=None, engine='igemm', dz=None):
         cm = cmult(self.dtype_code)
         assert x.is_cuda and x.is_contiguous() and x.dim() == 5 and x.shape[-1] == cm * self.cin_pad, \
             (tuple(x.shape), self.cin_pad)
@@ -365,7 +418,8 @@
             off, strides = out_view[:2]
             os_lo = out_view[2] if len(out_view) > 2 else 0
             assert code != _lib.DTYPE_BF16X2 or os_lo > 0, 'a split output view needs its hi -> lo offset'
-        p = self.params(N, iD, iH, iW, strides, code, cout_store, os_lo)
+        p = self.params(N, iD, iH, iW, strides, code, cout_store, os_lo, dz)
+        p.dz_planes = None if plane_counter is None else plane_counter.data_ptr()
         L = _lib.load()
         fn = L.s3d_conv_igemm if engine == 'igemm' else L.s3d_conv_direct
         esz = out.element_size()
diff --git a/stereo_3d_reconstruction_b200/lib.py b/stereo_3d_reconstruction_b200/lib.py
--- a/stereo_3d_reconstruction_b200/lib.py
+++ b/stereo_3d_reconstruction_b200/lib.py
@@ -29,6 +29,8 @@
         ('bn', ctypes.c_int32),
         ('proj_w', ctypes.c_void_p), ('proj_channel', ctypes.c_int32), ('proj_act', ctypes.c_int32),
         ('w_nstack', ctypes.c_void_p),
+        ('dz_nref', ctypes.c_int32), ('dz_c', ctypes.c_int32), ('dz_e', ctypes.c_int32), ('dz_pairs', ctypes.c_int32),
+        ('dz_sched', ctypes.c_void_p), ('dz_planes', ctypes.c_void_p),
     ]
 
 
@@ -107,7 +109,7 @@
 
 HOST_KNOBS = ('no_vol2d', 'no_concat_fuse', 'no_cls_fused', 'no_conv_first', 'no_d2s', 'no_ref_once', 'no_cls_chain', 'no_sheared', 'no_map_conv', 'no_conv2d_halo')
 LIB_KNOBS = ('no_scatter', 'scatter_tps3', 'scatter_no_pair', 'scatter_ring', 'scatter_res_transpose',
-             'scatter_no_transpose', 'scatter_generic', 'no_corr_tc', 'scatter_zsplit', 'scatter_no_rm', 'igemm_ts1', 'igemm_one_cta', 'scatter_one_cta', 'no_conv_first_tc', 'chamfer_sym', 'chamfer_sym_r')
+             'scatter_no_transpose', 'scatter_generic', 'no_corr_tc', 'scatter_zsplit', 'scatter_no_rm', 'igemm_ts1', 'igemm_one_cta', 'scatter_one_cta', 'no_conv_first_tc', 'chamfer_sym', 'chamfer_sym_r', 'no_dz_skip')
 KNOBS = {k: int(os.environ.get('S3D_' + k.upper()) is not None) for k in HOST_KNOBS}
 KNOBS['no_scatter'] = int(os.environ.get('S3D_NO_SCATTER') is not None)
 
diff --git a/stereo_3d_reconstruction_b200/models.py b/stereo_3d_reconstruction_b200/models.py
--- a/stereo_3d_reconstruction_b200/models.py
+++ b/stereo_3d_reconstruction_b200/models.py
@@ -299,9 +299,10 @@
                 assert feat.shape[-1] == cm * C, 'FEAT_CHANNELS must be a multiple of 16'
                 vol = ops.cost_volume_concat(feat, B, D, out=self._buf('vol', (2 * B, D, h, w, 2 * cm * C), dt), split=self._split)
                 a = self._conv('dres0a', vol, out=self._bufo('a0', 'dres0a', vol))
-            a = self._conv('dres0b', a, out=self._bufo('a1', 'dres0b', a))
-            y = self._conv('dres1a', a, out=self._bufo('a2', 'dres1a', a))
-            a = self._conv('dres1b', y, residual=a, out=self._bufo('a3', 'dres1b', y))
+            bf = self.precision == 'bf16'
+            a = self._conv('dres0b', a, out=self._bufo('a1', 'dres0b', a), dz=(B, 3, 1) if bf else None)
+            y = self._conv('dres1a', a, out=self._bufo('a2', 'dres1a', a), dz=(B, 5, 2) if bf else None)
+            a = self._conv('dres1b', y, residual=a, out=self._bufo('a3', 'dres1b', y), dz=(B, 7, 3) if bf else None)
             S = self._packed['cls_b'].cout_pad
             pa = self._packed['cls_a']
             if (self.precision == 'bf16' and isinstance(pa, PackedConv) and pa.weight_ns is not None and pa.cin_pad == 64 and
```

Result: faster. 5133 (median of 6 runs) (+3.4%).
